# kemingy/rabitq

Measured on AMD Instinct MI355X. Metric: queries/sec at recall@10>=0.95, 100Mx128; HBM GB/s on popcount scan, higher is better.
Workload: dtype exact integer dot (fp6 MFMA, v_dot8_u32_u4) + f32

## Files before the change

### rabitq_amd/csrc/host_query.h

```cpp
#pragma once
struct QueryParams {
    uint32_t nq, len, probe, topk;
    bool heuristic;
    uint32_t cap, hcap;
    const float *thr_init = nullptr;
    bool seg_final = false;
    bool ext_lists = false;
    const rq_filter *filter = nullptr;
};

#define RQ_DEFAULT_CAP 4096u
#define RQ_MAX_CAP_HINT 32768u
#define RQ_MAX_NQ_PER_PASS 65536u
#define RQ_MAX_PROBE 16384u

static rq_status ws_prepare(const rq_index *idx, Workspace &ws, const QueryParams &qp) {
    const uint32_t nprobe = std::min(qp.probe, idx->k);
    const uint64_t nq = qp.nq, npairs = nq * nprobe;
    if (!ws.stream) HIPC(hipStreamCreateWithFlags(&ws.stream, hipStreamNonBlocking));
    if (!ws.h_totals) HIPC(hipHostMalloc((void **)&ws.h_totals, 16 * sizeof(unsigned long long)));
    RQC(ws.qpad.ensure(nq * idx->dim));
    RQC(ws.y.ensure(nq * idx->dim));
    if (!qp.ext_lists) RQC(ws.dist.ensure(nq * idx->k));
    RQC(ws.probe_dist.ensure(npairs));
// ... 21 lines not shown
    RQC(ws.heap_key.ensure(nq * qp.topk));
    RQC(ws.heap_id.ensure(nq * qp.topk));
    RQC(ws.precise.ensure(nq));
    RQC(ws.need.ensure(nq));
    RQC(ws.ovf.ensure(nq));
    RQC(ws.q_cap.ensure(nq));
    RQC(ws.q_base.ensure(nq));
    RQC(ws.nsurv.ensure(nq));
    RQC(ws.nshadow.ensure(nq));
    RQC(ws.recent.ensure(nq));
    RQC(ws.win_count.ensure(nq));
    RQC(ws.arr_len.ensure(nq));
    RQC(ws.row_map.ensure(nq));
    RQC(ws.big_list.ensure(nq + 3));
    if (qp.heuristic) RQC(ws.arr.ensure(nq * qp.hcap));
    return RQ_OK;
}

struct PassResult {
    uint64_t rough = 0, precise = 0, overflowed = 0, max_need = 0;
};

static rq_status finish_pass(const rq_index *idx, Workspace &ws, PassResult *res, rq_profile_t *prof_acc) {
    Prof &pf = ws.prof;
    const uint32_t nq = ws.pend_nq, dim = idx->dim;
    HIPC(hipStreamSynchronize(ws.stream));
    HIPC(hipGetLastError());
    res->rough = ws.h_totals[0];
    res->precise = ws.h_totals[1];
    res->overflowed = ws.h_totals[2];
    res->max_need = ws.h_totals[4];
    if (rq_large_batch(nq)) hints_of(idx, ws.pend_filter).big_dirs.store((uint32_t)ws.h_totals[7]);
    if (ws.pend_additive && ws.h_totals[8] >= 4096 && ws.h_totals[9] * 32 > ws.h_totals[8])
        const_cast<rq_index *>(idx)->additive_loose.store(1);
    if (prof_acc) prof_acc->matrix_subtile_steps += ws.h_totals[8], prof_acc->matrix_exact_steps += ws.h_totals[9];
    if (prof_acc) prof_acc->coarse_fallback_rows += (uint32_t)std::min<unsigned long long>(ws.h_totals[10], 0xFFFFFFFFull);
    if (pf.on && prof_acc) {
        float ms[PF_N] = {0};
        pf.collect(ms);
        prof_acc->ms_rotate += ms[PF_ROTATE], prof_acc->ms_coarse += ms[PF_COARSE];
        prof_acc->ms_select += ms[PF_SELECT], prof_acc->ms_prep += ms[PF_PREP], prof_acc->ms_group += ms[PF_GROUP];
        prof_acc->ms_scan += ms[PF_SCAN] + ms[PF_SCAN_MATRIX], prof_acc->ms_scan_matrix += ms[PF_SCAN_MATRIX];
        prof_acc->ms_rerank += ms[PF_RERANK], prof_acc->ms_sort += ms[PF_SORT];
        if (!ws.pend_matrix_ranges.empty()) {
            std::vector<unsigned long long> len(nq);
            HIPC(hipMemcpy(len.data(), ws.pend_filter ? ws.stream_len.p : ws.rough_cnt.p, (size_t)nq * 8, hipMemcpyDeviceToHost));
            for (const StreamRange &r : ws.pend_matrix_ranges)
                for (uint32_t b = 0; b < nq; ++b)
                    prof_acc->matrix_pairs += std::min<unsigned long long>(len[b], r.s_hi) - std::min<unsigned long long>(len[b], r.s_lo);
        }
        prof_acc->ms_replay += ms[PF_REPLAY], prof_acc->ms_total += ms[PF_TOTAL], prof_acc->ms_early += ms[PF_EARLY];
    }
    if (prof_acc) {
        const uint64_t slots = std::max<uint64_t>((uint64_t)nq * ws.pend_cap, ws.pend_seg_slots);
        prof_acc->survivor_workspace_bytes = std::max<uint64_t>(prof_acc->survivor_workspace_bytes,
            ws.pend_seg_slots ? (ws.surv.count + ws.runs.count + ws.runs_tmp.count + ws.arena_recs.count + ws.arena_runs.count) * 16ull
                              : slots * (ws.use_runs_tmp ? 48ull : 32ull));
        prof_acc->segmented_passes += ws.pend_seg_slots ? 1u : 0u;
        prof_acc->scan_candidates += res->rough;
        prof_acc->scan_bytes += res->rough * (uint64_t)(dim / 8 + 16);
        prof_acc->rerank_candidates += ws.h_totals[3];
        prof_acc->rerank_shadow_rejects += ws.h_totals[5];
        if (g_scan_dbg.load() & 256) {
            unsigned long long ht[12];
            HIPC(hipMemcpy(ht, ws.stat.p + 128, sizeof ht, hipMemcpyDeviceToHost));
            if (ht[3])
                fprintf(stderr, "[rabitq_hip] scan_mfma exact path (wave 0 of every block): %.0f cycles per block inside it (of which flushes %.0f), "
                        "%.1f flagged registers, %.1f with survivors and %.2f flushes per block\n", (double)ht[5] / ht[3], (double)ht[6] / ht[3],
                        (double)ht[9] / ht[3], (double)ht[7] / ht[3], (double)ht[8] / ht[3]);
            if (ht[3])
                fprintf(stderr, "[rabitq_hip] scan_mfma timing: %llu blocks, %.1f tiles/block; per block cycles: start-up %.0f, "
                        "tile-loop waits %.0f, tile bodies %.0f (per tile: wait %.0f, body %.0f)\n", ht[3], (double)ht[4] / ht[3],
                        (double)ht[0] / ht[3], (double)ht[1] / ht[3], (double)ht[2] / ht[3], (double)ht[1] / std::max(1ull, ht[4]),
                        (double)ht[2] / std::max(1ull, ht[4]));
        }
        if ((g_scan_dbg.load() & 4096) && nq <= RQ_SB_MAX_NQ) {
            unsigned long long hs[32];
            HIPC(hipMemcpy(hs, ws.stat.p, sizeof hs, hipMemcpyDeviceToHost));
            std::string line = "[rabitq_hip] sb_query_kernel phases (us since entry):";
            for (unsigned long long i = 1; i < std::min<unsigned long long>(hs[0], 30); ++i) line += " " + std::to_string((hs[1 + i] - hs[1]) / 100.0).substr(0, 6);
            fprintf(stderr, "%s\n", line.c_str());
        }
    }
    return RQ_OK;
}

static rq_status run_pass(const rq_index *idx, Workspace &ws, const float *d_q, const QueryParams &qp,
                          const uint32_t *d_row_map, float *d_out_dist, uint32_t *d_out_id, uint32_t *d_out_n,
                          PassResult *res, rq_profile_t *prof_acc, const uint32_t *ext_cluster = nullptr,
                          const float *ext_dist = nullptr, bool defer = false) {
    const uint32_t dim = idx->dim, k = idx->k, W = idx->W;
    const uint32_t nq = qp.nq, nprobe = std::min(qp.probe, k), topk = qp.topk;
    const uint32_t npairs = nq * nprobe;
    bool listed = false;
    uint32_t nlive = 0;
    const rq_filter *filt = qp.filter;
    ws.pend_filter = filt;
    const uint32_t min_len = filt ? 0u : idx->min_list_len;
    hipStream_t st = ws.stream;
    ws.pend_prefiltered = false;
    Prof &pf = ws.prof;
    pf.reset(g_profiling.load(), st);
    pf.begin(PF_TOTAL);
    size_t total_span = pf.spans.size() ? pf.spans.size() - 1 : 0;

    const int impl = g_scan_impl.load();
    struct Stage {
        uint32_t s_lo, s_hi;
    };
    auto build_stages = [&](uint64_t first_hi, uint64_t growth, uint64_t settle_cap) {
        std::vector<Stage> stages;
        const uint64_t total_max = std::min<uint64_t>((uint64_t)nprobe * idx->max_list_len, idx->n);
        uint64_t lo = 0, hi = first_hi;
        const uint64_t avg = std::max<uint64_t>(1, idx->n / std::max<uint32_t>(idx->nonempty_lists, 1));
        uint64_t settle = std::min(settle_cap, std::max<uint64_t>(avg, std::min<uint64_t>(idx->max_list_len, 16 * avg)));
        if (rq_large_batch(nq)) settle = std::max<uint64_t>(1, settle * (uint64_t)g_stage_settle_pct.load() / 100);
        while (lo < total_max) {
            const bool last = hi >= total_max || lo >= settle;
            stages.push_back({(uint32_t)lo, last ? 0xFFFFFFFFu : (uint32_t)hi});
            if (last) break;
            lo = hi;
            hi = std::min<uint64_t>(hi * growth, 0xFFFFFFF0ull);
            if (lo < 2 * avg && 2 * hi > 2 * avg) hi = 2 * avg;
            if (lo < settle && hi > settle) hi = settle;
        }
        return stages;
    };
    std::vector<Stage> stages;
    ReplayState rs;
    rs.thr = ws.thr.p, rs.heap_len = ws.heap_len.p, rs.heap_key = ws.heap_key.p, rs.heap_id = ws.heap_id.p;
    rs.precise = ws.precise.p, rs.need = ws.need.p, rs.nsurv = ws.nsurv.p, rs.nshadow = ws.nshadow.p, rs.recent_max = ws.recent.p, rs.win_count = ws.win_count.p;
    rs.arr_len = ws.arr_len.p, rs.arr = ws.arr.p, rs.hcap = qp.hcap;
    rs.ovf = ws.ovf.p;
    const QSeg useg{nullptr, nullptr, qp.cap};
    const float *qpad = d_q;
    const uint32_t *probe_cluster = ws.probe_cluster.p;
    const float *probe_dist = ws.probe_dist.p;
    const uint32_t *rerank_order = nullptr;
    const bool one_stage = qp.thr_init != nullptr && d_row_map == nullptr;
    auto stage_on_matrix = [&](const Stage &sg) {
        const uint64_t avg_len = std::max<uint64_t>(1, idx->n / std::max<uint32_t>(idx->nonempty_lists, 1));
        const uint64_t span = (uint64_t)std::min<uint64_t>(sg.s_hi, (uint64_t)nprobe * idx->max_list_len) - sg.s_lo;
        const uint64_t est_pairs = (uint64_t)nq * std::min<uint64_t>(nprobe, span / avg_len + 2);
        return scan_has_mfma(W) && impl != 1 &&
               (impl == 2 || (est_pairs >= 8ull * k && (sg.s_lo >= avg_len * (uint64_t)g_stage_settle_pct.load() / 100 || one_stage)));
    };

    const bool sb_w = W == 1 || W == 2 || W == 4 || W == 8 || W == 12 || W == 16;
    bool small = g_small_batch.load() == 0 && nq <= RQ_SB_MAX_NQ && !ext_cluster && !d_row_map && !qp.thr_init && !filt && sb_w &&
                 k <= RQ_SB_MAX_K && nprobe <= 64 && topk <= RQ_SB_MAX_TOPK && qp.cap <= 4 * RQ_DEFAULT_CAP;
    bool sb_results_done = false;
    bool sb_fused_finish = false;
    bool sb_filled = false;
    if (small) {
        const int gopt = g_stage_growth.load();
        stages = build_stages(16ull * std::max<uint32_t>(topk, 1), gopt >= 2 ? (uint64_t)gopt : 8, (uint64_t)std::max(1, g_sb_span.load()));
        if (stages.size() > RQ_SB_MAX_STAGES) small = false;
    }
    if (small) {
        const uint64_t total_max = std::min<uint64_t>((uint64_t)nprobe * idx->max_list_len, idx->n);
        SbArgs sa{};
        const bool whole = stages.empty() || (total_max - stages.back().s_lo) * (uint64_t)(dim / 8 + 16) <= (1ull << 20);
        sa.nstages = (uint32_t)(whole ? stages.size() : stages.size() - 1);
        for (uint32_t i = 0; i < sa.nstages; ++i) sa.s_lo[i] = stages[i].s_lo, sa.s_hi[i] = stages[i].s_hi;
        const Stage fin = whole ? Stage{0, 0} : stages.back();
        const uint64_t fin_pairs = (uint64_t)nq * nprobe;
        const bool fin_cluster_major = !whole && fin_pairs >= k / 2 && fin_pairs > 64;
        sa.finalize = whole ? 1u : 0u;
        sa.fill_final = !whole && !fin_cluster_major ? 1u : 0u;
        sa.final_lo = fin.s_lo;
        sa.codes = reinterpret_cast<const uint32_t *>(idx->codes.p), sa.factors = idx->factors.p, sa.centroids = idx->centroids.p;
        sa.offsets = idx->offsets.p, sa.map_ids = idx->map_ids.p, sa.base = idx->view();
        sa.dist = ws.dist.p, sa.y = ws.y.p, sa.qpad = ws.qpad.p, sa.probe_cluster = ws.probe_cluster.p, sa.probe_dist = ws.probe_dist.p;
        sa.qf6 = scan_has_mfma(W) && impl != 1 ? ws.qf6.p : nullptr;
        sa.scal = ws.scal.p, sa.qnib = ws.qnib.p, sa.rough_cnt = ws.rough_cnt.p, sa.surv_cnt = ws.surv_cnt.p, sa.totals = ws.totals.p;
        sa.rs = rs, sa.out_dist = d_out_dist, sa.out_id = d_out_id, sa.out_n = d_out_n, sa.recs = ws.recs.p, sa.fs = idx->fstats;
        sa.k = k, sa.dim = dim, sa.nprobe = nprobe, sa.topk = topk, sa.cap = qp.cap, sa.hcap = qp.hcap;
        sa.stamps = (g_scan_dbg.load() & 4096) ? ws.stat.p : nullptr;
        if (sa.stamps) HIPC(hipMemsetAsync(ws.stat.p, 0, 8, st));
        else HIPC(hipMemsetAsync(ws.stat.p, 0, 256 * sizeof(unsigned long long), st));
        pf.begin(PF_COARSE);
        sb_front_kernel<<<dim3(ceil_div(k, RQ_SB_LISTS), ceil_div(nq, RQ_SB_QT)), 256, (size_t)2 * RQ_SB_QT * dim * sizeof(float), st>>>(
            d_q, qp.len, idx->P.p, idx->centroids.p, ws.y.p, ws.qpad.p, ws.dist.p, k, dim, nq, ws.totals.p, ws.big_list.p + nq);
        pf.end();
        pf.begin(PF_EARLY);
        const size_t dyn = (size_t)RQ_SB_CAP * sizeof(SurvRec) + (size_t)dim * 4 + (size_t)topk * 16;
        const int mode = qp.heuristic ? 2 : (topk < 64 ? 1 : 0);
#define RQ_SBQ(WW)                                                                        \
    do {                                                                                  \
        if (mode == 2) sb_query_kernel<WW, 2><<<nq, 1024, dyn, st>>>(sa);                 \
        else if (mode == 1) sb_query_kernel<WW, 1><<<nq, 1024, dyn, st>>>(sa);            \
        else sb_query_kernel<WW, 0><<<nq, 1024, dyn, st>>>(sa);                           \
    } while (0)
        switch (W) {
            case 1: RQ_SBQ(1); break;
            case 2: RQ_SBQ(2); break;
            case 4: RQ_SBQ(4); break;
            case 8: RQ_SBQ(8); break;
            case 12: RQ_SBQ(12); break;
            default: RQ_SBQ(16); break;
        }
#undef RQ_SBQ
        pf.end();
        qpad = ws.qpad.p;
        sb_results_done = whole && !qp.heuristic;
        sb_fused_finish = !whole && !qp.heuristic;
        sb_filled = sa.fill_final != 0;
        stages.clear();
        if (!whole) stages.push_back(fin);
        if (prof_acc) prof_acc->small_batch_passes++;
    } else {
    pf.begin(PF_ROTATE);
    if (qp.len != dim) {
        pad_rows_kernel<<<ceil_div((uint64_t)nq * dim, 256), 256, 0, st>>>(d_q, ws.qpad.p, nq, qp.len, dim);
        qpad = ws.qpad.p;
    }
    launch_rotate(qpad, idx->P.p, ws.y.p, nq, dim, nq >= 32, st);
    pf.end();

    if (ext_cluster) {
        probe_cluster = ext_cluster;
        probe_dist = ext_dist;
    } else {
        if (coarse_prefilter_applies(idx, nq, nprobe)) {
            pf.begin(PF_COARSE);
            HIPC(hipMemsetAsync(ws.totals.p + 12, 0, 8, st));
            RQC(ws.coarse_redo.ensure(nq));
            RQC(ws.qf6.ensure((size_t)nq * dim / 2 + 16));
            launch_coarse_prefiltered(idx, ws.y.p, ws.dist.p, nq, nprobe, ws.probe_cluster.p, ws.probe_dist.p, nprobe, ws.totals.p + 12, ws.coarse_redo.p, st,
                                      reinterpret_cast<uint16_t *>(ws.qf6.p));
            ws.pend_prefiltered = true;
            pf.end();
        } else {
            pf.begin(PF_COARSE);
            launch_coarse(idx->cent_t.p, ws.y.p, ws.dist.p, k, dim, nq, k, st);
            pf.end();
            pf.begin(PF_SELECT);
            launch_select(ws.dist.p, k, nprobe, ws.probe_cluster.p, ws.probe_dist.p, 0, nprobe, nq, st);
            pf.end();
        }
    }

    if (one_stage) {
        stages.push_back({0u, 0xFFFFFFFFu});
    } else {
        const int gopt = g_stage_growth.load();
        const uint64_t growth = gopt >= 2 ? (uint64_t)gopt : (nq >= 32768 ? 8 : 16);
        stages = build_stages((uint64_t)std::max<uint32_t>(topk, 1) * (rq_large_batch(nq) ? growth : 1), growth, ~0ull);
    }
    pf.begin(PF_PREP);
    {
        uint32_t *qn = scan_is_fused(W) ? ws.qnib.p : nullptr;
        uint32_t *q6 = scan_has_mfma(W) && impl != 1 ? ws.qf6.p : nullptr;
        uint32_t qn_slots = nprobe;
        if (qn && q6 && !ext_cluster && min_len > 0) {
            uint32_t reach = 0;
            for (const Stage &sg : stages)
                if (!stage_on_matrix(sg))
                    reach = std::max<uint32_t>(reach, sg.s_hi == 0xFFFFFFFFu ? nprobe : (uint32_t)std::min<uint64_t>(nprobe, (uint64_t)(sg.s_hi - 1) / min_len + 1));
            qn_slots = reach;
        }
        listed = (filt || (idx->nonempty_lists * 2 < k && npairs >= 65536)) && g_pair_split.load() != 0 &&
                 (dim == 64 || dim == 128 || dim == 256 || dim == 512 || dim == 768 || dim == 1024);
        if (listed) {
            RQC(ws.live_list.ensure((size_t)npairs + 1));
            HIPC(hipMemsetAsync(ws.live_list.p + npairs, 0, 4, st));
            pair_split_kernel<<<ceil_div(npairs, 4096), 1024, 0, st>>>(filt ? filt->sub_off.p : idx->offsets.p, probe_cluster, probe_dist, npairs,
                                                                       nprobe, k, ws.scal.p, ws.live_list.p, ws.live_list.p + npairs);
            unsigned long long *h_live = ws.h_totals + 15;
            *h_live = 0;
            HIPC(hipMemcpyAsync(h_live, ws.live_list.p + npairs, 4, hipMemcpyDeviceToHost, st));
            HIPC(hipStreamSynchronize(st));
            nlive = (uint32_t)*h_live;
        }
#define RQ_PREP_SMALL(LP, R, PPB, PP)                                                                              \
    do {                                                                                                           \
        if (listed)                                                                                                \
            prep_small_listed_kernel<LP, R, PP><<<std::max(1u, ceil_div(nlive, (PPB) * (PP))), 256, 0, st>>>(ws.y.p, idx->centroids.p, idx->offsets.p, probe_cluster, \
                                                                    probe_dist, ws.live_list.p, nlive, nprobe, ws.scal.p, qn, q6, k); \
        else                                                                                                       \
            prep_small_kernel<LP, R, PP><<<ceil_div(npairs, (PPB) * (PP)), 256, 0, st>>>(ws.y.p, idx->centroids.p, idx->offsets.p, probe_cluster, \
                                                                    probe_dist, npairs, nprobe, ws.scal.p, qn, q6, k, idx->nonempty_lists * 2 < k ? 2u : 1u, qn_slots); \
    } while (0)
        if (dim == 128) RQ_PREP_SMALL(16, 2, 16, 2);
        else if (dim == 64) RQ_PREP_SMALL(16, 1, 16, 4);
        else if (dim == 256) RQ_PREP_SMALL(32, 2, 8, 2);
        else if (dim == 512) RQ_PREP_SMALL(32, 4, 8, 1);
        else if (dim == 768) RQ_PREP_SMALL(32, 6, 8, 1);
        else if (dim == 1024) RQ_PREP_SMALL(32, 8, 8, 1);
#undef RQ_PREP_SMALL
        else
            prep_kernel<<<ceil_div(npairs, 4), 256, 0, st>>>(ws.y.p, idx->centroids.p, idx->offsets.p, probe_cluster, probe_dist,
                                                             npairs, nprobe, dim, ws.scal.p,
                                                             scan_is_fused(W) ? nullptr : ws.planes.p,
                                                             qn, q6, nullptr, k, 1u);
    }
    if (filt) {
        RQC(ws.stream_len.ensure(nq));
        pair_prefix_filtered_kernel<<<ceil_div(nq, 4), 256, 0, st>>>(ws.scal.p, nq, nprobe, ws.rough_cnt.p, probe_cluster, filt->sub_off.p, k,
                                                                     ws.stream_len.p);
    } else
        pair_prefix_kernel<<<ceil_div(nq, 4), 256, 0, st>>>(ws.scal.p, nq, nprobe, ws.rough_cnt.p);
    if (rq_large_batch(nq)) {
        HIPC(hipMemsetAsync(ws.q_hist.p, 0, (size_t)(k + 2) * 4, st));
        order_count_kernel<<<ceil_div(nq, 256), 256, 0, st>>>(probe_cluster, nprobe, nq, k, ws.q_hist.p);
        group_scan_kernel<<<1, 1024, 0, st>>>(ws.q_hist.p, k + 1, ws.q_start.p, 0u, nullptr, 0u);
        order_scatter_kernel<<<ceil_div(nq, 256), 256, 0, st>>>(probe_cluster, nprobe, nq, k, ws.q_start.p, ws.q_hist.p,
                                                                ws.q_order.p);
        rerank_order = ws.q_order.p;
    }
    init_state_kernel<<<ceil_div(nq, 256), 256, 0, st>>>(rs, ws.surv_cnt.p, nq, qp.thr_init, d_row_map);
    HIPC(hipMemsetAsync(ws.totals.p, 0, 8 * sizeof(unsigned long long), st));
    HIPC(hipMemsetAsync(ws.big_list.p + nq, 0, 12, st));
    HIPC(hipMemsetAsync(ws.stat.p, 0, 256 * sizeof(unsigned long long), st));
    pf.end();

    }
    ws.pend_matrix_ranges.clear();
    ws.pend_seg_slots = 0;
    ws.pend_additive = false, ws.pend_matrix_stages = 0;
    const uint32_t big_hint = hints_of(idx, filt).big_dirs.load();
    const uint32_t mid_blocks = big_hint == 0 ? 64u : std::min(4096u, std::max(256u, big_hint / 4));
    const uint32_t tile = scan_tile(W);
    const uint64_t avg_len = std::max<uint64_t>(1, idx->n / std::max<uint32_t>(idx->nonempty_lists, 1));
    uint32_t stage_no = ~0u;
    for (const Stage &sg : stages) {
        ++stage_no;
        const uint64_t span = (uint64_t)std::min<uint64_t>(sg.s_hi, (uint64_t)nprobe * idx->max_list_len) - sg.s_lo;
        const uint64_t est_pairs = (uint64_t)nq * std::min<uint64_t>(nprobe, span / avg_len + 2);
        const bool use_mfma = stage_on_matrix(sg);
        const bool cluster_major = use_mfma || (est_pairs >= k / (small ? 2u : (uint32_t)g_cluster_major_div.load()) && est_pairs > 64);
        if (g_scan_dbg.load() & 16384)
            fprintf(stderr, "[rabitq_hip] stage %u: [%u, %u) span %llu est_pairs %llu %s\n", stage_no, sg.s_lo, sg.s_hi,
                    (unsigned long long)span, (unsigned long long)est_pairs, use_mfma ? "matrix cores" : (cluster_major ? "VALU, list-major" : "VALU, pair-major"));
        const bool fp6_records = use_mfma;
        const bool arena_stage = qp.seg_final && span > qp.cap && scan_is_fused(W) && rq_large_batch(nq);
        const int gate_opt = g_scan_gate.load();
        const bool additive = use_mfma && !arena_stage && !filt && scan_has_additive(W) && idx->list_uref.p != nullptr && gate_opt != 1 &&
                              (gate_opt == 2 || !idx->additive_loose.load());
        pf.begin(PF_GROUP);
        ScanArgs a{};
        ScanPtrs sp{};
        a.cluster_major = cluster_major ? 1u : 0u;
        uint32_t slot_hi = nprobe;
        if (cluster_major && min_len > 0 && !ext_cluster && sg.s_hi != 0xFFFFFFFFu)
            slot_hi = (uint32_t)std::min<uint64_t>(nprobe, (uint64_t)(sg.s_hi - 1) / min_len + 1);
        const uint32_t stage_pairs = nq * slot_hi;
        bool ranked = false;
        if (cluster_major) {
            HIPC(hipMemsetAsync(ws.grp_cnt.p, 0, (size_t)((k + 4) & ~3u) * 4, st));
            const int rank_opt = g_group_rank.load();
            ranked = k <= 32768 && (rank_opt == 2 || (rank_opt == 1 && stage_pairs >= 16 * RQ_RANK_ITEMS &&
                                                      stage_pairs / RQ_RANK_ITEMS >= k / 256));
            if (ranked) {
                const uint32_t nblk = ceil_div(stage_pairs, RQ_RANK_ITEMS);
                RQC(ws.pair_rank.ensure(stage_pairs));
                RQC(ws.rank_base.ensure((size_t)nblk * k));
                group_rank_kernel<<<nblk, 1024, (size_t)k * 4, st>>>(ws.scal.p, probe_cluster, stage_pairs, nprobe, slot_hi, sg.s_lo,
                                                                    sg.s_hi, k, ws.grp_cnt.p, ws.pair_rank.p, ws.rank_base.p);
            } else
                group_count_kernel<<<ceil_div(stage_pairs, 256), 256, 0, st>>>(ws.scal.p, probe_cluster, stage_pairs, nprobe,
                                                                               slot_hi, sg.s_lo, sg.s_hi, ws.grp_cnt.p);
            group_scan_kernel<<<1, 1024, 0, st>>>(ws.grp_cnt.p, k, ws.grp_start.p, (use_mfma ? 1u : 0u) | (ranked ? 2u : 0u) | (additive ? 4u : 0u), ws.recs.p, 12 * W);
            a.ngroups = k;
        } else {
            a.ngroups = npairs;
        }
        const uint32_t *operand = fp6_records ? ws.qf6.p
                                              : (scan_is_fused(W) ? ws.qnib.p : reinterpret_cast<const uint32_t *>(ws.planes.p));
        if (!(sb_filled && !cluster_major)) {
            const bool fill_listed = listed && ranked && cluster_major && slot_hi == nprobe;
            const uint32_t fill_items = fill_listed ? nlive : stage_pairs;
            const bool fill8 = !use_mfma || additive;
            if (fill_items) {
                if (fill8)
                    stage_fill_kernel<8><<<ceil_div(fill_items, 32), 256, 0, st>>>(ws.scal.p, probe_cluster, operand, ws.thr.p, fill_items,
                                                                    nprobe, slot_hi, fp6_records ? 12 * W : 8 * W, sg.s_lo, sg.s_hi,
                                                                    a.cluster_major, ws.grp_start.p, ws.grp_cnt.p, ws.recs.p,
                                                                    idx->fstats, use_mfma ? (additive ? 2u : 1u) : 0u, ranked ? ws.pair_rank.p : nullptr,
                                                                    ws.rank_base.p, k, idx->list_uref.p, fill_listed ? ws.live_list.p : nullptr);
                else
                    stage_fill_kernel<16><<<ceil_div(fill_items, 16), 256, 0, st>>>(ws.scal.p, probe_cluster, operand, ws.thr.p, fill_items,
                                                                    nprobe, slot_hi, fp6_records ? 12 * W : 8 * W, sg.s_lo, sg.s_hi,
                                                                    a.cluster_major, ws.grp_start.p, ws.grp_cnt.p, ws.recs.p,
                                                                    idx->fstats, use_mfma ? (additive ? 2u : 1u) : 0u, ranked ? ws.pair_rank.p : nullptr,
                                                                    ws.rank_base.p, k, idx->list_uref.p, fill_listed ? ws.live_list.p : nullptr);
            }
        }
        if (additive) {
            RQC(ws.grp_vref.ensure(2 * (size_t)k));
            group_vrange_kernel<<<k, 256, 0, st>>>(ws.recs.p, ws.grp_start.p, ws.grp_cnt.p, 12 * W, ws.grp_vref.p);
            ws.pend_additive = true;
        }
        pf.end();
        sp.codes = reinterpret_cast<const uint32_t *>(idx->codes.p);
        sp.factors = idx->factors.p;
        sp.grp_start = ws.grp_start.p;
        sp.grp_cnt = ws.grp_cnt.p;
        sp.offsets = idx->offsets.p;
        sp.recs = ws.recs.p;
        sp.surv = ws.surv.p;
        sp.runs = ws.runs.p;
        sp.surv_cnt = ws.surv_cnt.p;
        sp.stat = ws.stat.p;
        sp.list_uref = idx->list_uref.p, sp.grp_vref = ws.grp_vref.p;
        sp.arena = arena_stage, sp.filtered = filt != nullptr;
        a.x = filt ? filt->extra.p : nullptr;
        a.cap = qp.cap;
        a.dbg = (uint32_t)g_scan_dbg.load();
        const uint32_t stage_tile = use_mfma ? scan_mfma_tile(W, arena_stage, additive) : tile;
        a.tiles_per_group = ceil_div(std::min<uint64_t>(idx->max_list_len, sg.s_hi), stage_tile);
        sp.tile_table = nullptr;
        const uint64_t grid_blocks = (uint64_t)k * a.tiles_per_group, real_tiles = idx->n / stage_tile + k;
        const int tt_opt = g_scan_tile_table.load();
        if (cluster_major && scan_is_fused(W) && sg.s_hi >= idx->max_list_len &&
            (tt_opt == 2 || (tt_opt == 1 && grid_blocks > 4 * real_tiles))) {
            uint32_t count = 0;
            sp.tile_table = get_tile_table(idx, stage_tile, &count);
            if (sp.tile_table) a.use_table = 1u, a.ngroups = count, a.tiles_per_group = 1u;
        }
        uint32_t dense_cells = 0;
        if (rq_large_batch(nq) && !use_mfma && scan_is_fused(W) && g_dense_dir.load() && sg.s_hi != 0xFFFFFFFFu &&
            !(qp.seg_final && span > qp.cap)) {
            const uint64_t cells = (uint64_t)((sg.s_hi - 1) >> 6) - (sg.s_lo >> 6) + 2ull * slot_hi + 2;
            if (cells <= qp.cap) dense_cells = (uint32_t)cells;
        }
        a.dense_dir = dense_cells ? 1u : 0u;
        QSeg seg = useg;
        bool runs_in_tmp = false;
        if (arena_stage) {
            uint64_t want = std::max<uint64_t>(hints_of(idx, filt).arena.load(), (uint64_t)nq * qp.cap / 2);
            unsigned long long total_slots = 0;
            uint32_t arena_rsub = 0;
            bool arena_retried = false;
            ws.arena_failed = true;
#ifdef RQ_DEV_ABLATIONS
            if (g_seg_opt.load() == 3) {
                DevBuf<SurvRec> never;
                RQC(never.alloc(1ull << 46));
                return fail(RQ_ERR_OOM, "survivor arena: injected failure (developer hook survivor_segments = 3)");
            }
#endif
            for (int attempt = 0;; ++attempt) {
                want = std::min<uint64_t>(want, 0xFFFF0000ull);
                RQC(ws.arena_recs.ensure(want));
                RQC(ws.arena_runs.ensure(want));
                RQC(ws.arena_cur.ensure(RQ_ARENA_SHARDS + 4));
                RQC(ws.arena_fail.ensure(RQ_ARENA_SHARDS));
                HIPC(hipMemsetAsync(ws.arena_cur.p, 0, (RQ_ARENA_SHARDS + 4) * 8, st));
                HIPC(hipMemsetAsync(ws.arena_fail.p, 0xFF, RQ_ARENA_SHARDS * 4, st));
                ScanExtra hx{};
                RQC(ws.arena_places.ensure(want));
                hx.arena_places = ws.arena_places.p, hx.allow = filt ? filt->pos_bits.p : nullptr;
                hx.arena_recs = ws.arena_recs.p, hx.arena_runs = reinterpret_cast<uint4 *>(ws.arena_runs.p), hx.arena_cur = ws.arena_cur.p;
                hx.arena_fail = ws.arena_fail.p;
                {
                    const uint64_t have = std::min<uint64_t>(ws.arena_recs.count, ws.arena_runs.count);
                    hx.arena_sub = hx.arena_rsub = (uint32_t)(have * 7 / 8 / RQ_ARENA_SHARDS);
                    hx.arena_common = (uint32_t)std::min<uint64_t>(have - (uint64_t)hx.arena_sub * RQ_ARENA_SHARDS, 0xFFFFFF00ull);
                }
                arena_rsub = hx.arena_rsub;
                RQC(ws.scan_extra.ensure(1));
                HIPC(hipMemcpyAsync(ws.scan_extra.p, &hx, sizeof hx, hipMemcpyHostToDevice, st));
                a.x = ws.scan_extra.p;
                a.dense_dir = 0u;
                pf.begin(use_mfma ? PF_SCAN_MATRIX : PF_SCAN);
                if (use_mfma) launch_scan_mfma(sp, a, W, st, additive);
                else launch_scan(sp, a, W, st);
                pf.end();
                pf.begin(PF_GROUP);
                seg_exact_kernel<<<ceil_div(nq, 256), 256, 0, st>>>(ws.surv_cnt.p, nq, 64u, ws.q_cap.p);
                seg_scan_kernel<<<1, 1024, 0, st>>>(ws.q_cap.p, nq, ws.q_base.p, ws.arena_cur.p + RQ_ARENA_SHARDS + 1);
                unsigned long long tail[2] = {0, 0};
                HIPC(hipMemcpyAsync(tail, ws.arena_cur.p + RQ_ARENA_SHARDS, 16, hipMemcpyDeviceToHost, st));
                HIPC(hipStreamSynchronize(st));
                total_slots = tail[1];
                if (!(uint32_t)tail[0]) break;
                pf.end();
                if (attempt >= 6 || want >= 0xFFFF0000ull) return fail(RQ_ERR_OOM, "survivor arena kept overflowing");
                const uint64_t nblocks = a.use_table ? a.ngroups : (uint64_t)a.ngroups * a.tiles_per_group;
                HIPC(hipMemsetAsync(ws.surv_cnt.p, 0, (size_t)nq * sizeof(unsigned long long), st));
                want = std::max<uint64_t>(want * 2, 1u << 20);
                if (nblocks < RQ_ARENA_SHARDS) want = std::max<uint64_t>(want, 8 * total_slots + (1u << 16)), arena_retried = true;
                else want = std::max<uint64_t>(want, total_slots + total_slots / 4);
            }
            ws.arena_failed = false;
            {
                std::atomic<uint64_t> &arena_hint = hints_of(idx, filt).arena;
                uint64_t cur = arena_hint.load();
                const uint64_t learnt = std::max<uint64_t>(total_slots + total_slots * 3 / 5, arena_retried ? std::min<uint64_t>(want, 0xFFFF0000ull) : 0ull);
                while (cur < learnt && !arena_hint.compare_exchange_weak(cur, learnt)) {}
            }
            if (total_slots > ws.surv.count || total_slots > ws.runs.count || total_slots > ws.runs_tmp.count) {
                const uint64_t grow = total_slots + total_slots / 8;
                RQC(ws.surv.ensure(grow));
                RQC(ws.runs.ensure(grow));
                RQC(ws.runs_tmp.ensure(grow));
            }
            sp.surv = ws.surv.p, sp.runs = ws.runs.p;
            arena_scatter_kernel<<<dim3(RQ_ARENA_SHARDS + RQ_ARENA_COMMON_BLOCKS, 2), 256, 0, st>>>(ws.arena_recs.p, reinterpret_cast<const uint4 *>(ws.arena_runs.p), ws.arena_cur.p,
                                                                              ws.arena_fail.p, arena_rsub, ws.q_base.p, ws.arena_places.p, ws.surv.p, ws.runs_tmp.p);
            runs_in_tmp = true;
            pf.end();
            seg = QSeg{ws.q_base.p, ws.q_cap.p, qp.cap};
            ws.pend_seg_slots = std::max<uint64_t>(ws.pend_seg_slots, total_slots);
        }
        if (dense_cells) {
            pf.begin(PF_SORT);
            clear_dir_kernel<<<ceil_div((uint64_t)nq * dense_cells, 256), 256, 0, st>>>(ws.runs.p, nq, seg, dense_cells);
            pf.end();
        }
        if (!arena_stage) {
            pf.begin(use_mfma ? PF_SCAN_MATRIX : PF_SCAN);
            if (use_mfma) launch_scan_mfma(sp, a, W, st, additive);
            else launch_scan(sp, a, W, st);
            pf.end();
        }
        if (use_mfma) ws.pend_matrix_stages++;
        if (prof_acc && additive) prof_acc->matrix_additive_launches++;
        if (prof_acc) prof_acc->scan_launches++;
        if (prof_acc && use_mfma) {
            prof_acc->matrix_launches++;
            ws.pend_matrix_ranges.push_back({sg.s_lo, sg.s_hi});
        }
        if (!rq_large_batch(nq) && qp.cap <= 4 * RQ_DEFAULT_CAP) {
            pf.begin(PF_RERANK);
            const uint32_t fin_threads = nq <= 16 ? 1024u : 256u;
            const uint32_t presorted = qp.cap > RQ_DEFAULT_CAP && nprobe <= 1024 ? 1u : 0u;
            if (presorted) {
                sort_runs_kernel<<<nq, 64, 0, st>>>(ws.runs.p, ws.surv_cnt.p, seg, ws.big_list.p, ws.big_list.p + nq, RQ_SORT_LDS_RECS, nullptr);
                sort_runs_mid_kernel<<<std::min(nq, 256u), 256, RQ_SORT_MID_LDS_WORDS * 8, st>>>(ws.runs.p, ws.use_runs_tmp ? ws.runs_tmp.p : nullptr, ws.surv_cnt.p,
                                                                                              seg, ws.big_list.p, ws.big_list.p + nq, nprobe, 0u,
                                                                                              RQ_SORT_MID_LDS_WORDS);
            }
            if (sb_fused_finish) {
                uint32_t flags = presorted;
                if (nq <= 32) {
                    accurate_kernel<<<dim3(std::max(1u, std::min(16u, 256u / nq)), nq), 256, (size_t)dim * sizeof(float), st>>>(
                        ws.surv.p, ws.surv_cnt.p, seg, idx->view(), qpad, dim, nullptr, probe_cluster, nprobe);
                    flags |= 2u;
                }
                const uint32_t presorted = flags;
                if (topk < 64)
                    sb_finish_kernel<true><<<nq, fin_threads, (size_t)dim * sizeof(float) + (2 * RQ_SBF_RUNS + RQ_SBF_RECS) * 16, st>>>(
                        ws.surv.p, ws.runs.p, ws.surv_cnt.p, seg, idx->view(), qpad, dim, topk, rs, probe_cluster, nprobe, presorted,
                        idx->map_ids.p, d_out_dist, d_out_id, d_out_n, ws.rough_cnt.p, ws.totals.p);
                else
                    sb_finish_kernel<false><<<nq, fin_threads, (size_t)dim * sizeof(float) + (2 * RQ_SBF_RUNS + RQ_SBF_RECS) * 16, st>>>(
                        ws.surv.p, ws.runs.p, ws.surv_cnt.p, seg, idx->view(), qpad, dim, topk, rs, probe_cluster, nprobe, presorted,
                        idx->map_ids.p, d_out_dist, d_out_id, d_out_n, ws.rough_cnt.p, ws.totals.p);
                sb_results_done = true;
            } else if (qp.heuristic)
                stage_finish_kernel<true><<<nq, fin_threads, (size_t)dim * sizeof(float), st>>>(ws.surv.p, ws.runs.p, ws.surv_cnt.p, seg, idx->view(),
// ... 462 lines not shown
```

### rabitq_amd/csrc/host_state.h

```cpp
#pragma once
static thread_local std::string g_err;
static rq_status fail(rq_status s, const std::string &msg) {
    g_err = msg;
    return s;
}
#define HIPC(expr)                                                                                   \
    do {                                                                                             \
        hipError_t _e = (expr);                                                                      \
        if (_e != hipSuccess)                                                                        \
            return fail(_e == hipErrorOutOfMemory ? RQ_ERR_OOM : RQ_ERR_HIP,                         \
                        std::string(#expr) + ": " + hipGetErrorString(_e));                          \
    } while (0)
#define RQC(expr)                        \
    do {                                 \
        rq_status _s = (expr);           \
        if (_s != RQ_OK) return _s;      \
    } while (0)

static rq_status ensure_device() {
    int count = 0;
    hipError_t e = hipGetDeviceCount(&count);
    if (e != hipSuccess || count == 0)
        return fail(RQ_ERR_NO_DEVICE, "no HIP device visible (librabitq_hip has no CPU fallback)");
    return RQ_OK;
}

template <typename T>
struct DevBuf {
    T *p = nullptr;
    size_t count = 0;
    DevBuf() = default;
    DevBuf(const DevBuf &) = delete;
    DevBuf &operator=(const DevBuf &) = delete;
    ~DevBuf() { release(); }
    void release() {
        if (p) (void)hipFree(p);
        p = nullptr;
        count = 0;
    }
    rq_status alloc(size_t n) {
        release();
        count = n;
        if (n == 0) n = 1;
        hipError_t e = hipMalloc((void **)&p, n * sizeof(T));
        if (e != hipSuccess) {
            p = nullptr;
            count = 0;
            return fail(RQ_ERR_OOM, "hipMalloc of " + std::to_string(n * sizeof(T)) + " bytes failed: " +
                                        hipGetErrorString(e));
        }
        return RQ_OK;
    }
    rq_status ensure(size_t n) { return n <= count && p ? RQ_OK : alloc(n); }
};

template <typename T>
static rq_status copy_out_sized(T *out, T full) {
    const uint32_t sz = out->struct_size;
    if (sz < 8) return fail(RQ_ERR_INVALID, "struct_size is not set (set it to sizeof(the struct) before the call)");
    const uint32_t w = std::min<uint32_t>(sz, (uint32_t)sizeof(T));
    full.struct_size = w;
    memcpy(out, &full, w);
    return RQ_OK;
}
static inline uint32_t ceil_div(uint64_t a, uint64_t b) { return (uint32_t)((a + b - 1) / b); }
template <int W, int NT>
static size_t assign_lds_bytes() { return 2 * (32 * (64 * W * 2 + 16) + 128); }
static inline uint32_t pow2_ceil(uint32_t v) {
    uint32_t p = 1;
    while (p < v) p <<= 1;
    return p;
}

static std::atomic<uint64_t> g_rough{0}, g_precise{0}, g_query{0}, g_miss{0};

enum { PF_ROTATE = 0, PF_COARSE, PF_SELECT, PF_PREP, PF_GROUP, PF_SCAN, PF_SCAN_MATRIX, PF_RERANK, PF_SORT, PF_REPLAY, PF_EARLY, PF_TOTAL, PF_N };
static std::atomic<int> g_profiling{0};
static thread_local rq_profile_t g_profile;

struct Prof {
    bool on = false;
    bool light = false;
    hipStream_t stream = nullptr;
    struct Span {
        hipEvent_t a, b;
        int cat;
    };
    std::vector<Span> spans;
    std::vector<hipEvent_t> pool;
    size_t used = 0;
    bool open = false;
    hipEvent_t last_b = nullptr;
    bool failed = false;
    hipEvent_t get() {
        if (used == pool.size()) {
            hipEvent_t e = nullptr;
            if (hipEventCreate(&e) != hipSuccess || !e) {
                failed = true;
                on = false;
                return nullptr;
            }
            pool.push_back(e);
        }
        return pool[used++];
    }
    void begin(int cat) {
        open = on && !(light && cat != PF_SCAN && cat != PF_SCAN_MATRIX && cat != PF_TOTAL);
        if (!open) {
            last_b = nullptr;
            return;
        }
        Span s{last_b, get(), cat};
        if (s.b && !s.a) {
            s.a = get();
            if (s.a) (void)hipEventRecord(s.a, stream);
        }
        last_b = nullptr;
        if (!s.a || !s.b) {
            open = false;
            spans.clear();
            return;
        }
        spans.push_back(s);
    }
    void end() {
        if (!open) return;
        (void)hipEventRecord(spans.back().b, stream);
        last_b = spans.back().b;
        open = false;
    }
    void reset(int level, hipStream_t st) {
        on = level != 0;
        light = level == 2;
        stream = st;
        spans.clear();
        used = 0;
        open = false;
        last_b = nullptr;
        failed = false;
    }
    void collect(float *ms ) {
        if (failed) return;
        for (auto &s : spans) {
            float t = 0;
            (void)hipEventElapsedTime(&t, s.a, s.b);
            ms[s.cat] += t;
        }
    }
    ~Prof() {
        for (auto e : pool) (void)hipEventDestroy(e);
    }
};

struct StreamRange {
    uint32_t s_lo, s_hi;
};
struct Workspace {
    hipStream_t stream = nullptr;
    bool busy = false;
    size_t pend_total_span = 0;
    uint64_t pend_seg_slots = 0;
    uint32_t pend_cap = 0;
    uint32_t pend_nq = 0;
    std::vector<StreamRange> pend_matrix_ranges;
    DevBuf<float> qpad, y, dist, probe_dist, thr, recent;
    DevBuf<float> retry_q, retry_pd, retry_pc;
    DevBuf<uint32_t> retry_rows;
    DevBuf<uint32_t> q_hist, q_start, q_order;
    DevBuf<uint32_t> live_list;
    DevBuf<uint32_t> coarse_redo;
    DevBuf<uint32_t> pair_rank, rank_base;
    DevBuf<uint32_t> probe_cluster, recs, grp_cnt, grp_start, heap_len, heap_id, precise, need,
        nsurv, nshadow, win_count, arr_len, row_map, big_list;
    DevBuf<int32_t> heap_key;
    DevBuf<PairScalars> scal;
    DevBuf<uint64_t> planes;
    DevBuf<uint32_t> qnib;
    DevBuf<uint32_t> qf6;
    DevBuf<unsigned long long> rough_cnt, totals, surv_cnt, stat;
    DevBuf<unsigned long long> stream_len;
    const struct rq_filter *pend_filter = nullptr;
    DevBuf<float4> grp_vref;
    bool pend_additive = false;
    uint32_t pend_matrix_stages = 0;
    bool pend_prefiltered = false;
    DevBuf<SurvRec> surv, arr;
    DevBuf<RunRec> runs, runs_tmp;
    bool use_runs_tmp = false;
    bool arena_failed = false;
    DevBuf<float> sh_dist;
    DevBuf<uint32_t> sh_id, sh_n;
    DevBuf<unsigned long long> sh_packed, sh_gathered, sh_merged;
    DevBuf<uint32_t> ovf, q_cap;
    DevBuf<unsigned long long> q_base;
    DevBuf<SurvRec> arena_recs;
    DevBuf<RunRec> arena_runs;
    DevBuf<uint2> arena_places;
    DevBuf<unsigned long long> arena_cur;
    DevBuf<unsigned int> arena_fail;
    DevBuf<ScanExtra> scan_extra;
    DevBuf<uint32_t> sh_flag;
    DevBuf<uint32_t> sh_pc, sh_id_b, sh_n_b;
    DevBuf<float> sh_pd, sh_thr, sh_dist_b;
    unsigned long long *h_totals = nullptr;
    Prof prof;
    ~Workspace() {
        if (h_totals) (void)hipHostFree(h_totals);
        if (stream) (void)hipStreamDestroy(stream);
    }
};

struct rq_index {
    uint32_t dim = 0, k = 0, W = 0, max_list_len = 0;
    uint32_t min_list_len = 0;
    uint64_t n = 0;
    uint64_t n_dev = 0;
    float *base_host = nullptr;
    float *base_host_dev = nullptr;
    DevBuf<ListTier> list_tier;
    std::vector<ListTier> h_list_tier;
    bool split_rows = false;
    BaseView view() const { return BaseView{base.p, base_host_dev, list_tier.p, k, split_rows ? 1u : 0u}; }
    ~rq_index() {
        if (base_host) (void)hipHostFree(base_host);
    }
    DevBuf<float> base, P, centroids, cent_t;
    DevBuf<_Float16> base_h;
    DevBuf<uint8_t> base_q8;
    DevBuf<float4> list_q8;
    DevBuf<uint32_t> offsets, map_ids;
    DevBuf<uint64_t> codes;
    DevBuf<float4> factors;
    DevBuf<float4> list_uref;
    DevBuf<uint16_t> cent_bf;
    DevBuf<float> cent_sqnorm;
    float cent_norm_max = INFINITY;
    uint32_t nonempty_lists = 0;
    std::atomic<int> additive_loose{0};
    std::mutex ws_mu;
    std::vector<std::unique_ptr<Workspace>> ws_pool;
    FactorStats fstats{0, 0, 0, 0};
    std::atomic<uint32_t> cap_hint{0};
    std::atomic<uint64_t> arena_hint{0};
    std::atomic<uint32_t> big_dirs_hint{0};
    uint64_t pass_budget = 24ull << 30;
    std::vector<uint32_t> h_offsets;
    std::mutex tt_mu;
    std::map<uint32_t, std::unique_ptr<DevBuf<uint4>>> tile_tables;
    DevBuf<uint32_t> row_key;
    bool row_key_valid = false;
    bool row_order_ok = true;
    bool is_shard = false;
    uint64_t generation = 0;
    std::atomic<int> open_tickets{0};
};

struct rq_filter {
    const rq_index *idx = nullptr;
    uint64_t generation = 0;
    DevBuf<uint32_t> pos_bits;
    DevBuf<uint32_t> sub_off;
    DevBuf<ScanExtra> extra;
    uint64_t rows = 0;
    std::atomic<uint32_t> cap_hint{0};
    std::atomic<uint64_t> arena_hint{0};
    std::atomic<uint32_t> big_dirs_hint{0};
};
struct PassHints {
    std::atomic<uint32_t> &cap;
    std::atomic<uint64_t> &arena;
    std::atomic<uint32_t> &big_dirs;
};
static PassHints hints_of(const rq_index *idx, const rq_filter *f) {
    if (f) {
        rq_filter *m = const_cast<rq_filter *>(f);
        return PassHints{m->cap_hint, m->arena_hint, m->big_dirs_hint};
    }
    rq_index *m = const_cast<rq_index *>(idx);
    return PassHints{m->cap_hint, m->arena_hint, m->big_dirs_hint};
}

__global__ void fill_f32_kernel(float *p, float v, uint64_t n) {
    uint64_t i = (uint64_t)blockIdx.x * blockDim.x + threadIdx.x;
    if (i < n) p[i] = v;
}
__global__ void gather_rows_kernel(const float *__restrict__ in, const uint32_t *__restrict__ rows,
                                   uint32_t nrows, uint32_t len, float *__restrict__ out) {
    uint64_t i = (uint64_t)blockIdx.x * blockDim.x + threadIdx.x;
    if (i >= (uint64_t)nrows * len) return;
    uint32_t r = (uint32_t)(i / len), c = (uint32_t)(i - (uint64_t)r * len);
    out[i] = in[(uint64_t)rows[r] * len + c];
}

__global__ __launch_bounds__(256) void shard_gather_kernel(const uint32_t *__restrict__ new_off, const uint32_t *__restrict__ old_off,
                                                           uint32_t k, uint64_t n_local, uint32_t dim,
                                                           const BaseView base_in, const uint64_t *__restrict__ codes_in,
                                                           const float4 *__restrict__ factors_in, const uint32_t *__restrict__ ids_in,
                                                           const BaseView base_out, uint64_t *__restrict__ codes_out,
                                                           float4 *__restrict__ factors_out, uint32_t *__restrict__ ids_out) {
    const uint32_t lane = threadIdx.x & 63, W = dim >> 6;
    for (uint64_t p = (uint64_t)blockIdx.x * 4 + (threadIdx.x >> 6); p < n_local; p += (uint64_t)gridDim.x * 4) {
        uint32_t lo = 0, hi = k;
        while (hi - lo > 1) {
            const uint32_t mid = lo + ((hi - lo) >> 1);
            if (new_off[mid] <= p) lo = mid;
            else hi = mid;
        }
        const uint64_t src = (uint64_t)old_off[lo] + (p - new_off[lo]);
        const RowRef srow = base_in.row(src, dim), drow = base_out.row(p, dim);
        for (uint32_t e = lane; e < dim; e += 64) rq_row_put(drow, dim, e, rq_row_get(srow, dim, e));
        for (uint32_t w = lane; w < W; w += 64) codes_out[p * W + w] = codes_in[src * W + w];
        if (lane == 0) {
            factors_out[p] = factors_in[src];
            ids_out[p] = ids_in[src];
        }
    }
}
__global__ void pack_topk_keys_kernel(const float *__restrict__ dist, const uint32_t *__restrict__ id, const uint32_t *__restrict__ cnt,
                                      uint32_t nq, uint32_t topk, uint32_t id_offset, unsigned long long *__restrict__ keys) {
    const uint64_t i = (uint64_t)blockIdx.x * blockDim.x + threadIdx.x;
    if (i >= (uint64_t)nq * topk) return;
    const uint32_t b = (uint32_t)(i / topk), e = (uint32_t)(i - (uint64_t)b * topk);
    keys[i] = e < cnt[b] ? (((unsigned long long)ord32_biased(dist[i]) << 32) | (uint32_t)(id[i] + id_offset)) : ~0ull;
}
// ... 57 lines not shown
                                                                                                    kstride);
}

static std::atomic<int> g_pair_split{1};
static std::atomic<int> g_coarse_tiled_from{4096};
static bool coarse_prefilter_has(uint32_t W) { return W == 1 || W == 2 || W == 3 || W == 4 || W == 6 || W == 8 || W == 12; }
static bool coarse_prefilter_applies(const rq_index *idx, uint32_t nq, uint32_t nprobe) {
    const int impl = g_coarse_impl.load();
    return (impl == 3 || impl == 4 || (impl == 0 && nq >= 2048)) && coarse_prefilter_has(idx->W) && std::isfinite(idx->cent_norm_max) &&
           idx->cent_bf.p != nullptr && nprobe <= 64 && nq >= 8 && idx->k >= 64 && nprobe >= 1 && idx->k <= 65536;
}
static void launch_coarse_prefiltered(const rq_index *idx, const float *y, float *dist, uint32_t nq, uint32_t nprobe, uint32_t *out_cluster,
                                      float *out_dist, uint32_t out_stride, unsigned long long *fallback_rows, uint32_t *redo, hipStream_t st,
                                      uint16_t *y_bf) {
    const uint32_t k = idx->k, dim = idx->dim;
    if (idx->W > 8) to_bf16_kernel<<<ceil_div((uint64_t)nq * dim / 8, 256), 256, 0, st>>>(y, (uint64_t)nq * dim, y_bf);
#define RQ_CAP(WW, NT)                                                                                                      \
    coarse_approx_kernel<WW, NT><<<ceil_div(nq, 128 * NT), 256, assign_lds_bytes<WW, NT>(), st>>>(y, idx->cent_bf.p, idx->cent_sqnorm.p, nq, \
                                                                                                  k, dist, y_bf)
    switch (idx->W) {
        case 1: RQ_CAP(1, 2); break;
        case 2: RQ_CAP(2, 2); break;
        case 3: RQ_CAP(3, 1); break;
        case 4: RQ_CAP(4, 1); break;
        case 6: RQ_CAP(6, 1); break;
        case 8: RQ_CAP(8, 1); break;
        default: RQ_CAP(12, 1); break;
    }
#undef RQ_CAP
    const dim3 g(ceil_div(nq, 4)), b(256);
    const uint32_t ntile = ceil_div(k, 32u);
    const int impl = g_coarse_impl.load();
    const bool tiled = redo != nullptr && ntile >= nprobe &&
                       (k > 8192 || impl == 4 || (impl != 3 && k >= (uint32_t)g_coarse_tiled_from.load() && idx->W <= 8));
    if (tiled) {
#define RQ_TILED(TPL)                                                                                                             \
    select_refine_tiled_kernel<TPL><<<g, b, 4 * 64 * (TPL) * 4, st>>>(dist, y, idx->centroids.p, idx->cent_norm_max, k, dim, nprobe, out_cluster, \
                                                                    out_dist, out_stride, nq, redo, fallback_rows)
        if (ntile <= 128) RQ_TILED(2);
        else if (ntile <= 256) RQ_TILED(4);
        else if (ntile <= 512) RQ_TILED(8);
        else if (ntile <= 1024) RQ_TILED(16);
        else RQ_TILED(32);
#undef RQ_TILED
        select_probe_kernel<<<nq, 256, (size_t)nprobe * 8, st>>>(dist, k, nprobe, out_cluster, out_dist, 0u, out_stride, redo);
    } else if (k <= 1024)
        select_refine_wave_kernel<16><<<g, b, 0, st>>>(dist, y, idx->centroids.p, idx->cent_norm_max, k, dim, nprobe, out_cluster, out_dist, out_stride, nq, fallback_rows);
    else if (k <= 4096)
        select_refine_wave_kernel<64><<<g, b, 0, st>>>(dist, y, idx->centroids.p, idx->cent_norm_max, k, dim, nprobe, out_cluster, out_dist, out_stride, nq, fallback_rows);
    else
        select_refine_wave_kernel<128><<<g, b, 0, st>>>(dist, y, idx->centroids.p, idx->cent_norm_max, k, dim, nprobe, out_cluster, out_dist, out_stride, nq, fallback_rows);
}

#define RQ_MAX_BLOCKS_256 ((1u << 23) - 1)

static void launch_rotate(const float *x, const float *P, float *out, uint64_t n, uint32_t dim, bool mfma,
                          hipStream_t st) {
    const uint64_t rows_per_launch = mfma ? (1ull << 40) : (uint64_t)RQ_MAX_BLOCKS_256 * 4;
    for (uint64_t r0 = 0; r0 < n; r0 += rows_per_launch) {
        const uint64_t m = std::min(rows_per_launch, n - r0);
        const float *xs = x + r0 * dim;
        float *os = out + r0 * dim;
        if (mfma) {
            const uint32_t ncol = dim / ROT_BN;
            const uint64_t nrow_tiles = ceil_div(m, ROT_BM);
            const uint32_t groups = (uint32_t)std::min<uint64_t>(nrow_tiles, std::max<uint32_t>(1, 512 / ncol));
            rotate_mfma_kernel<<<dim3(groups * ncol), dim3(256), 0, st>>>(xs, P, os, m, dim, groups);
        } else {
            rotate_valu_kernel<<<dim3(ceil_div(m, 4), dim / 64), dim3(64, 4), 0, st>>>(xs, P, os, m, dim);
        }
    }
}

static const uint4 *get_tile_table(const rq_index *cidx, uint32_t tile, uint32_t *count) {
    rq_index *idx = const_cast<rq_index *>(cidx);
    std::lock_guard<std::mutex> lk(idx->tt_mu);
    auto it = idx->tile_tables.find(tile);
    if (it == idx->tile_tables.end()) {
        std::vector<uint4> h;
        h.reserve(idx->n / tile + idx->k + 1);
        for (uint32_t c = 0; c < idx->k; ++c) {
            const uint32_t b = idx->h_offsets[c], len = idx->h_offsets[c + 1] - b;
            for (uint32_t f = 0; f < len; f += tile) h.push_back(make_uint4(c, f, b, len));
        }
        std::unique_ptr<DevBuf<uint4>> buf(new DevBuf<uint4>());
        if (buf->alloc(h.size()) != RQ_OK) return nullptr;
        if (!h.empty() && hipMemcpy(buf->p, h.data(), h.size() * sizeof(uint4), hipMemcpyHostToDevice) != hipSuccess) return nullptr;
        buf->count = h.size();
        it = idx->tile_tables.emplace(tile, std::move(buf)).first;
    }
    *count = (uint32_t)it->second->count;
    return it->second->p;
}

static std::atomic<uint32_t> g_max_scan_blocks{RQ_MAX_BLOCKS_256};
template <typename F>
static void launch_scan_chunks(const ScanArgs &a, F &&launch) {
    if (a.ngroups == 0 || a.tiles_per_group == 0) return;
    const uint32_t maxb = std::max(1u, g_max_scan_blocks.load());
    const uint32_t tchunk = std::min(a.tiles_per_group, maxb);
    const uint32_t gchunk = std::max(1u, maxb / tchunk);
    for (uint32_t t0 = 0; t0 < a.tiles_per_group; t0 += tchunk)
        for (uint32_t g0 = 0; g0 < a.ngroups; g0 += gchunk) {
            ScanArgs c = a;
            c.tile_base = t0, c.group_base = g0;
            c.tiles_per_group = std::min(tchunk, a.tiles_per_group - t0);
            c.ngroups = std::min(gchunk, a.ngroups - g0);
            launch(c, dim3(c.ngroups * c.tiles_per_group));
        }
}

#define SCAN_ARGS p.codes, p.factors, p.offsets, p.grp_start, p.recs, p.surv, p.runs, p.surv_cnt, p.tile_table, a
template <bool ARENA, bool FILT>
static void launch_scan_t(const ScanPtrs &p, const ScanArgs &args, uint32_t W, hipStream_t st) {
    launch_scan_chunks(args, [&](const ScanArgs &a, dim3 g) {
        const dim3 b(256);
#define RQ_SCAN_K(WW, CPL)                                                                        \
    do {                                                                                          \
        if constexpr (FILT) scan_kernel<WW, CPL, ARENA, true><<<g, b, 0, st>>>(SCAN_ARGS);         \
        else scan_kernel<WW, CPL, ARENA><<<g, b, 0, st>>>(SCAN_ARGS);                             \
    } while (0)
        switch (W) {
            case 1: RQ_SCAN_K(1, 2); break;
            case 2: RQ_SCAN_K(2, 2); break;
            case 3: RQ_SCAN_K(3, 2); break;
            case 4: RQ_SCAN_K(4, 2); break;
            case 6: RQ_SCAN_K(6, 2); break;
            case 8: RQ_SCAN_K(8, 2); break;
            case 12: RQ_SCAN_K(12, 1); break;
            case 16: RQ_SCAN_K(16, 1); break;
            default:
                if constexpr (!ARENA && FILT) scan_generic_filtered_kernel<<<g, b, 0, st>>>(SCAN_ARGS, W);
                else if constexpr (!ARENA) scan_generic_kernel<<<g, b, 0, st>>>(SCAN_ARGS, W);
                break;
        }
#undef RQ_SCAN_K
    });
}
static void launch_scan(const ScanPtrs &p, const ScanArgs &args, uint32_t W, hipStream_t st) {
    if (p.filtered) {
        if (p.arena) launch_scan_t<true, true>(p, args, W, st);
        else launch_scan_t<false, true>(p, args, W, st);
    } else if (p.arena) launch_scan_t<true, false>(p, args, W, st);
    else launch_scan_t<false, false>(p, args, W, st);
}
static std::atomic<int> g_scan_impl{0};
static std::atomic<int> g_scan_gate{0};
static std::atomic<int> g_stage_growth{0};
static std::atomic<int> g_large_from{256};
static bool rq_large_batch(uint32_t nq) { return nq >= (uint32_t)g_large_from.load(); }
static std::atomic<int> g_cluster_major_div{32};
static std::atomic<int> g_stage_settle_pct{100};
static std::atomic<int> g_scan_tile_table{1};
static std::atomic<int> g_group_rank{1};
static std::atomic<int> g_shared_thr{1};
static std::atomic<int> g_sb_span{2560};
static std::atomic<int> g_seg_opt{1};
static std::atomic<int> g_pass_overlap{1};
static std::atomic<int> g_small_batch{0};
static std::atomic<int> g_dense_dir{1};

static bool scan_has_mfma(uint32_t W) {
    switch (W) {
        case 1: case 2: case 3: case 4: case 6: case 8: case 12: case 16: return true;
        default: return false;
    }
}
static uint32_t scan_mfma_nt(uint32_t W, bool additive = false) { return W == 2 ? (additive ? RQ_ADD_NT2 : RQ_NT_W2) : (W == 12 ? RQ_NT_W12 : (W >= 4 ? 2 : 4)); }
static uint32_t scan_mfma_nw(uint32_t W, bool arena) { return W == 2 && !arena ? 8u : 4u; }
static uint32_t scan_mfma_tile(uint32_t W, bool arena, bool additive = false) { return 32 * scan_mfma_nw(W, arena) * scan_mfma_nt(W, additive && !arena); }
static size_t scan_mfma_ring_bytes(uint32_t W, bool arena = false) {
    (void)arena;
    const uint64_t slots = W <= 2 ? 4ull : (W >= 16 ? 5ull : 3ull);
    return slots * (32 * (12 * W + 2) + RQ_REC_TAIL * 32) * 4;
}
template <int W, int NT, bool ARENA, bool ADD = false, bool FILT = false>
static void launch_scan_mfma_t(const ScanPtrs &p, const ScanArgs &a, dim3 g, hipStream_t st) {
    scan_mfma_kernel<W, NT, ARENA, ADD, FILT><<<g, dim3(64 * scan_mfma_waves<W, ARENA>()), scan_mfma_ring_bytes(W, ARENA), st>>>(p.codes, p.factors, p.offsets, p.grp_start, p.grp_cnt,
                                                                                    p.recs, p.surv, p.runs, p.surv_cnt, p.stat, p.tile_table, p.list_uref, p.grp_vref, a);
}
static bool scan_has_additive(uint32_t W) { return W == 1 || W == 2; }
static void launch_scan_mfma_add(const ScanPtrs &p, const ScanArgs &args, uint32_t W, hipStream_t st) {
    launch_scan_chunks(args, [&](const ScanArgs &a, dim3 g) {
        switch (W) {
            case 1: launch_scan_mfma_t<1, 4, false, true>(p, a, g, st); break;
            case 2: launch_scan_mfma_t<2, RQ_ADD_NT2, false, true>(p, a, g, st); break;
            default: break;
        }
    });
}
template <bool ARENA, bool FILT = false>
static void launch_scan_mfma_a(const ScanPtrs &p, const ScanArgs &args, uint32_t W, hipStream_t st) {
    launch_scan_chunks(args, [&](const ScanArgs &a, dim3 g) {
        switch (W) {
            case 1: launch_scan_mfma_t<1, 4, ARENA, false, FILT>(p, a, g, st); break;
            case 2: launch_scan_mfma_t<2, RQ_NT_W2, ARENA, false, FILT>(p, a, g, st); break;
            case 3: launch_scan_mfma_t<3, 4, ARENA, false, FILT>(p, a, g, st); break;
            case 4: launch_scan_mfma_t<4, 2, ARENA, false, FILT>(p, a, g, st); break;
            case 6: launch_scan_mfma_t<6, 2, ARENA, false, FILT>(p, a, g, st); break;
            case 8: launch_scan_mfma_t<8, 2, ARENA, false, FILT>(p, a, g, st); break;
            case 12: launch_scan_mfma_t<12, RQ_NT_W12, ARENA, false, FILT>(p, a, g, st); break;
            case 16: launch_scan_mfma_t<16, 2, ARENA, false, FILT>(p, a, g, st); break;
            default: break;
        }
    });
}
static void launch_scan_mfma(const ScanPtrs &p, const ScanArgs &args, uint32_t W, hipStream_t st, bool additive = false) {
    if (p.filtered) {
        if (p.arena) launch_scan_mfma_a<true, true>(p, args, W, st);
        else launch_scan_mfma_a<false, true>(p, args, W, st);
    } else if (p.arena) launch_scan_mfma_a<true>(p, args, W, st);
    else if (additive) launch_scan_mfma_add(p, args, W, st);
    else launch_scan_mfma_a<false>(p, args, W, st);
}

static bool scan_is_fused(uint32_t W) {
    switch (W) {
        case 1: case 2: case 3: case 4: case 6: case 8: case 12: case 16: return true;
        default: return false;
    }
}
static uint32_t scan_tile(uint32_t W) {
    switch (W) {
        case 1: case 2: case 3: case 4: case 6: case 8: return 512;
        default: return 256;
    }
}

static void launch_select(const float *dist, uint32_t k, uint32_t nprobe, uint32_t *out_cluster, float *out_dist,
                          uint32_t id_offset, uint32_t out_stride, uint32_t nq, hipStream_t st) {
    if (select_is_wave(k, nprobe, nq)) {
        const dim3 g(ceil_div(nq, 4)), b(256);
        if (k <= 1024) select_probe_wave_kernel<16><<<g, b, 0, st>>>(dist, k, nprobe, out_cluster, out_dist, id_offset, out_stride, nq);
        else if (k <= 4096) select_probe_wave_kernel<64><<<g, b, 0, st>>>(dist, k, nprobe, out_cluster, out_dist, id_offset, out_stride, nq);
        else select_probe_wave_kernel<128><<<g, b, 0, st>>>(dist, k, nprobe, out_cluster, out_dist, id_offset, out_stride, nq);
        return;
    }
    select_probe_kernel<<<nq, 256, (size_t)nprobe * 8, st>>>(dist, k, nprobe, out_cluster, out_dist, id_offset, out_stride);
}

template <int W, int NT>
static hipError_t set_scan_mfma_attr() {
    hipError_t e = hipFuncSetAttribute(reinterpret_cast<const void *>(scan_mfma_kernel<W, NT, false>),
                                       hipFuncAttributeMaxDynamicSharedMemorySize, (int)scan_mfma_ring_bytes(W));
    if (e != hipSuccess) return e;
    if constexpr (W <= 2) {
        e = hipFuncSetAttribute(reinterpret_cast<const void *>(scan_mfma_kernel<W, (W == 2 ? RQ_ADD_NT2 : NT), false, true>),
                                hipFuncAttributeMaxDynamicSharedMemorySize, (int)scan_mfma_ring_bytes(W));
        if (e != hipSuccess) return e;
    }
    e = hipFuncSetAttribute(reinterpret_cast<const void *>(scan_mfma_kernel<W, NT, true>),
                            hipFuncAttributeMaxDynamicSharedMemorySize, (int)scan_mfma_ring_bytes(W));
    if (e != hipSuccess) return e;
    e = hipFuncSetAttribute(reinterpret_cast<const void *>(scan_mfma_kernel<W, NT, false, false, true>),
                            hipFuncAttributeMaxDynamicSharedMemorySize, (int)scan_mfma_ring_bytes(W));
    if (e != hipSuccess) return e;
    return hipFuncSetAttribute(reinterpret_cast<const void *>(scan_mfma_kernel<W, NT, true, false, true>),
                               hipFuncAttributeMaxDynamicSharedMemorySize, (int)scan_mfma_ring_bytes(W));
}
static rq_status ensure_kernel_attributes() {
    static std::once_flag once;
    static hipError_t err = hipSuccess;
    static const char *what = "";
    std::call_once(once, [] {
        auto set = [&](const void *fn, int bytes, const char *name) {
            if (err != hipSuccess) return;
            err = hipFuncSetAttribute(fn, hipFuncAttributeMaxDynamicSharedMemorySize, bytes);
            if (err != hipSuccess) what = name;
        };
        set(reinterpret_cast<const void *>(select_probe_kernel), 140 * 1024, "select_probe_kernel");
        set(reinterpret_cast<const void *>(coarse_dist_kernel<4>), 140 * 1024, "coarse_dist_kernel<4>");
        set(reinterpret_cast<const void *>(coarse_dist_kernel<8>), 140 * 1024, "coarse_dist_kernel<8>");
        set(reinterpret_cast<const void *>(assign_generic_kernel<8>), 140 * 1024, "assign_generic_kernel<8>");
        set(reinterpret_cast<const void *>(merge_smallest_u64_kernel), 16384 * 8, "merge_smallest_u64_kernel");
        set(reinterpret_cast<const void *>(group_rank_kernel), 32768 * 4, "group_rank_kernel");
        set(reinterpret_cast<const void *>(sb_front_kernel), 140 * 1024, "sb_front_kernel");
        set(reinterpret_cast<const void *>(sort_runs_mid_kernel), RQ_SORT_MID_LDS_WORDS * 8, "sort_runs_mid_kernel");
        set(reinterpret_cast<const void *>(assign_approx_kernel<6, 1>), (int)assign_lds_bytes<6, 1>(), "assign_approx_kernel<6,1>");
        set(reinterpret_cast<const void *>(assign_approx_kernel<8, 1>), (int)assign_lds_bytes<8, 1>(), "assign_approx_kernel<8,1>");
        set(reinterpret_cast<const void *>(assign_approx_kernel<12, 1>), (int)assign_lds_bytes<12, 1>(), "assign_approx_kernel<12,1>");
        set(reinterpret_cast<const void *>(coarse_approx_kernel<6, 1>), (int)assign_lds_bytes<6, 1>(), "coarse_approx_kernel<6,1>");
        set(reinterpret_cast<const void *>(coarse_approx_kernel<8, 1>), (int)assign_lds_bytes<8, 1>(), "coarse_approx_kernel<8,1>");
        set(reinterpret_cast<const void *>(coarse_approx_kernel<12, 1>), (int)assign_lds_bytes<12, 1>(), "coarse_approx_kernel<12,1>");
        set(reinterpret_cast<const void *>(sb_finish_kernel<true>), 104 * 1024, "sb_finish_kernel");
        set(reinterpret_cast<const void *>(sb_finish_kernel<false>), 104 * 1024, "sb_finish_kernel");
#define RQ_SBQ_ATTR(WW)                                                                                  \
    set(reinterpret_cast<const void *>(sb_query_kernel<WW, 0>), 120 * 1024, "sb_query_kernel");          \
    set(reinterpret_cast<const void *>(sb_query_kernel<WW, 1>), 120 * 1024, "sb_query_kernel");          \
    set(reinterpret_cast<const void *>(sb_query_kernel<WW, 2>), 120 * 1024, "sb_query_kernel")
        RQ_SBQ_ATTR(1);
        RQ_SBQ_ATTR(2);
        RQ_SBQ_ATTR(4);
        RQ_SBQ_ATTR(8);
        RQ_SBQ_ATTR(12);
        RQ_SBQ_ATTR(16);
#undef RQ_SBQ_ATTR
        auto chk = [&](hipError_t e, const char *name) {
            if (err == hipSuccess && e != hipSuccess) err = e, what = name;
        };
        chk(set_scan_mfma_attr<1, 4>(), "scan_mfma_kernel<1,4>");
        chk(set_scan_mfma_attr<2, RQ_NT_W2>(), "scan_mfma_kernel<2,NT>");
        chk(set_scan_mfma_attr<3, 4>(), "scan_mfma_kernel<3,4>");
        chk(set_scan_mfma_attr<4, 2>(), "scan_mfma_kernel<4,2>");
        chk(set_scan_mfma_attr<6, 2>(), "scan_mfma_kernel<6,2>");
        chk(set_scan_mfma_attr<8, 2>(), "scan_mfma_kernel<8,2>");
        chk(set_scan_mfma_attr<12, RQ_NT_W12>(), "scan_mfma_kernel<12,NT>");
// ... 8 lines not shown
```

### rabitq_amd/csrc/kernels_query.h

```cpp
#pragma once
#ifndef RQ_COLLECT_UNROLL
#define RQ_COLLECT_UNROLL 8
#endif
#include "common.h"
#include "kernels_scan_common.h"

#pragma clang fp contract(off)

__global__ void pad_rows_kernel(const float *__restrict__ in, float *__restrict__ out, uint64_t n,
                                uint32_t len, uint32_t dim) {
    uint64_t i = (uint64_t)blockIdx.x * blockDim.x + threadIdx.x;
    if (i >= n * dim) return;
    uint64_t r = i / dim;
    uint32_t c = (uint32_t)(i - r * dim);
    out[i] = c < len ? in[r * len + c] : 0.0f;
}

__global__ __launch_bounds__(256) void rotate_valu_kernel(const float *__restrict__ x,
                                                          const float *__restrict__ P,
                                                          float *__restrict__ out, uint64_t n,
                                                          uint32_t dim) {
    uint64_t r = (uint64_t)blockIdx.x * 4 + threadIdx.y;
    uint32_t j = blockIdx.y * 64 + threadIdx.x;
    if (r >= n) return;
// ... 694 lines not shown
                for (int i = 0; i < (int)(RQ_COARSE_CAND / 64); ++i) c += (uint32_t)__popcll(__ballot(kk[i] <= mid));
                if (c >= nprobe) {
                    h2 = mid;
                    if (c <= nprobe + 12) break;
                } else {
                    l2 = mid + 1;
                }
            }
            T2 = coarse_margin_key(yr, dim, cmax, ord32_unbias(h2));
            ok = T2 != 0xFFFFFFFFu && collect(T2);
        }
    }
    if (!ok || base < nprobe) {
        for (uint32_t j0 = 0; j0 < k; j0 += 32) {
            uint32_t jj[4];
            float ee[4];
#pragma unroll
            for (int q = 0; q < 4; ++q) jj[q] = j0 + 8 * q + grp < k ? j0 + 8 * q + grp : 0u;
            coarse_exact_dist4(centroids, yr, dim, al, jj, ee);
#pragma unroll
            for (int q = 0; q < 4; ++q)
                if (j0 + 8 * q + grp < k && al == 0) d[j0 + 8 * q + grp] = ee[q];
        }
        if (lane == 0) {
            redo_flag[b] = 1u;
            if (fallback_rows) atomicAdd(fallback_rows, 1ull);
        }
        return;
    }
    if (lane == 0) redo_flag[b] = 0u;
    __builtin_amdgcn_fence(__ATOMIC_SEQ_CST, "wavefront");
    coarse_refine_tail(wn, base, centroids, yr, dim, nprobe, b, out_cluster, out_dist, out_stride);
}

__global__ __launch_bounds__(256) void merge_smallest_u64_kernel(const unsigned long long *__restrict__ in, uint32_t world,
                                                                 uint32_t nq, uint32_t width, uint32_t m_out,
                                                                 unsigned long long *__restrict__ out, uint64_t rank_stride) {
    extern __shared__ __attribute__((aligned(16))) unsigned char merge_smem[];
    unsigned long long *keys = reinterpret_cast<unsigned long long *>(merge_smem);
    const uint32_t b = blockIdx.x, m = world * width;
    for (uint32_t i = threadIdx.x; i < m; i += blockDim.x) {
        const uint32_t w = i / width, e = i - w * width;
        keys[i] = in[(uint64_t)w * rank_stride + (uint64_t)b * width + e];
    }
    __syncthreads();
    bitonic_sort_block(keys, m, [](unsigned long long v) { return v; });
    for (uint32_t i = threadIdx.x; i < m_out; i += blockDim.x) out[(uint64_t)b * m_out + i] = i < m ? keys[i] : ~0ull;
}

__global__ __launch_bounds__(256) void prep_kernel(const float *__restrict__ y,
                                                   const float *__restrict__ centroids,
                                                   const uint32_t *__restrict__ offsets,
                                                   const uint32_t *__restrict__ pair_cluster,
                                                   const float *__restrict__ pair_ycd, uint32_t npairs,
                                                   uint32_t pairs_per_row, uint32_t dim,
                                                   PairScalars *__restrict__ scal,
                                                   uint64_t *__restrict__ planes,
                                                   uint32_t *__restrict__ qnib,
                                                   uint32_t *__restrict__ qf6,
                                                   uint32_t *__restrict__ out_sum_u32, uint32_t nlists,
                                                   uint32_t skip_empty) {
    const uint32_t lane = threadIdx.x & 63;
    const uint32_t p = blockIdx.x * 4 + (threadIdx.x >> 6);
    if (p >= npairs) return;
    const uint32_t row = p / pairs_per_row;
    const uint32_t c = pair_cluster[p];
    const uint32_t len_c = c < nlists ? offsets[c + 1] - offsets[c] : 0u;
    if (len_c == 0 && skip_empty) {
        if (lane == 0) {
            PairScalars s;
            s.lower = 0.0f, s.delta = 0.0f, s.sumq = 0.0f, s.ycd = pair_ycd[p], s.ycd_sqrt = 0.0f;
            s.row = row, s.list_begin = 0, s.list_len = 0, s.stream_begin = 0, s.pad = 0;
            scal[p] = s;
            if (out_sum_u32) out_sum_u32[p] = 0;
        }
        return;
    }
    const float *yr = y + (uint64_t)row * dim;
    const float *cr = centroids + (uint64_t)c * dim;
    const uint32_t W = dim >> 6;
    float mn = 3.402823466e+38f, mx = -3.402823466e+38f;
    for (uint32_t w = 0; w < W; ++w) {
        float r = yr[64 * w + lane] - cr[64 * w + lane];
        mn = r < mn ? r : mn;
        mx = r > mx ? r : mx;
    }
    for (int o = 32; o >= 1; o >>= 1) {
        float a = __shfl_xor(mn, o, 64), bb = __shfl_xor(mx, o, 64);
        mn = a < mn ? a : mn;
        mx = bb > mx ? bb : mx;
    }
    const float scalar = 1.0f / 15.0f;
    const float delta = (mx - mn) * scalar;
    const float one_over_delta = 1.0f / delta;
    uint32_t sum = 0;
    uint64_t *pl = planes + (uint64_t)p * 4 * W;
    for (uint32_t w = 0; w < W; ++w) {
        float r = yr[64 * w + lane] - cr[64 * w + lane];
        int32_t q = cvtps_epi32((r - mn) * one_over_delta);
        sum += (uint32_t)q;
        if (planes) {
#pragma unroll
            for (int bit = 0; bit < 4; ++bit) {
                uint64_t word = __ballot((q >> bit) & 1);
                if (lane == 0) pl[bit * W + w] = word;
            }
        }
        if (qf6) {
            const uint32_t v = (uint32_t)q & 15u;
            const uint32_t c6 = v < 4 ? 4 * v : (v < 8 ? 8 + 2 * v : 16 + v);
            const uint32_t i16 = lane & 15, bitpos = 6 * i16, d0 = bitpos >> 5, off = bitpos & 31;
            const uint64_t wide = (uint64_t)c6 << off;
            const uint32_t lo32 = (uint32_t)wide, hi32 = (uint32_t)(wide >> 32);
            uint32_t w0 = d0 == 0 ? lo32 : 0u;
            uint32_t w1 = d0 == 0 ? hi32 : (d0 == 1 ? lo32 : 0u);
            uint32_t w2 = d0 == 1 ? hi32 : (d0 == 2 ? lo32 : 0u);
#pragma unroll
            for (int o = 1; o < 16; o <<= 1) {
                w0 |= __shfl_xor(w0, o, 16);
                w1 |= __shfl_xor(w1, o, 16);
                w2 |= __shfl_xor(w2, o, 16);
            }
            if (i16 < 3)
                qf6[(uint64_t)p * 12 * W + (lane >> 5) * 6 * W + 6 * w + 3 * ((lane >> 4) & 1) + i16] =
                    i16 == 0 ? w0 : (i16 == 1 ? w1 : w2);
        }
        if (qnib) {
            uint32_t nib = ((uint32_t)q & 15u) << (4 * (lane & 7));
            nib |= __shfl_xor(nib, 1, 8);
            nib |= __shfl_xor(nib, 2, 8);
            nib |= __shfl_xor(nib, 4, 8);
            if ((lane & 7) == 0) qnib[(uint64_t)p * 8 * W + 8 * w + (lane >> 3)] = nib;
        }
    }
    for (int o = 32; o >= 1; o >>= 1) sum += __shfl_xor(sum, o, 64);
    if (lane == 0) {
        PairScalars s;
        float ycd = pair_ycd[p];
        s.lower = mn;
        s.delta = delta;
        s.sumq = (float)sum;
        s.ycd = ycd;
        s.ycd_sqrt = sqrtf(ycd);
        s.row = row;
        s.list_begin = offsets[c];
        s.list_len = offsets[c + 1] - offsets[c];
        s.stream_begin = 0;
        s.pad = 0;
        scal[p] = s;
        if (out_sum_u32) out_sum_u32[p] = sum;
    }
}

template <int LP, int R, int PP>
__device__ __forceinline__ void prep_small_pairs(const float *__restrict__ y, const float *__restrict__ centroids,
                                                 const uint32_t *__restrict__ offsets,
                                                 const uint32_t *__restrict__ pair_cluster,
                                                 const float *__restrict__ pair_ycd, uint32_t npairs,
                                                 uint32_t pairs_per_row, PairScalars *__restrict__ scal,
                                                 uint32_t *__restrict__ qnib, uint32_t *__restrict__ qf6,
                                                 uint32_t nlists, uint32_t skip_empty, uint32_t p0,
                                                 const uint32_t *__restrict__ live_list = nullptr ,
                                                 uint32_t qn_slots = 0xFFFFFFFFu ) {
    static_assert(R >= 1 && (LP == 16 || LP == 32 || LP == 64), "lane groups of 16 / 32 / 64; a round = 4 LP dimensions (the packing's neighbour exchanges stay inside a round)");
    constexpr uint32_t DIM = 4 * LP * R, W = DIM / 64, PPW = 64 / LP;
    const uint32_t lane = threadIdx.x & 63, sub = lane % LP;
    uint32_t cl[PP], lb[PP], ll[PP];
    float ycd_in[PP];
    bool live[PP];
    uint32_t pid[PP];
#pragma unroll
    for (int pp = 0; pp < PP; ++pp) {
        const uint32_t pi = p0 + pp * PPW;
        live[pp] = pi < npairs;
        pid[pp] = live_list ? (live[pp] ? live_list[pi] : 0u) : pi;
        const uint32_t p = pid[pp];
        cl[pp] = live[pp] ? pair_cluster[p] : 0xFFFFFFFFu;
        ycd_in[pp] = live[pp] ? pair_ycd[p] : 0.0f;
    }
    float4 cv[PP][R], yv[PP][R];
#pragma unroll
    for (int pp = 0; pp < PP; ++pp) {
        const uint32_t p = pid[pp], c = cl[pp];
        const bool in = live[pp] && c < nlists;
        lb[pp] = in ? offsets[c] : 0u;
        ll[pp] = in ? offsets[c + 1] - lb[pp] : 0u;
        const uint32_t row = live[pp] ? p / pairs_per_row : 0u;
        const bool fetch = skip_empty == 2 ? ll[pp] != 0 : true;
#pragma unroll
        for (int rd = 0; rd < R; ++rd) {
            if (fetch) {
                yv[pp][rd] = *reinterpret_cast<const float4 *>(y + (uint64_t)row * DIM + 4 * LP * rd + 4 * sub);
                cv[pp][rd] = *reinterpret_cast<const float4 *>(centroids + (uint64_t)(in ? c : 0u) * DIM + 4 * LP * rd + 4 * sub);
            } else {
                yv[pp][rd] = make_float4(0.0f, 0.0f, 0.0f, 0.0f), cv[pp][rd] = make_float4(0.0f, 0.0f, 0.0f, 0.0f);
            }
        }
    }
#pragma unroll
    for (int pp = 0; pp < PP; ++pp) {
        const uint32_t p = pid[pp];
        if (!live[pp]) continue;
        const uint32_t row = p / pairs_per_row;
        if (ll[pp] == 0 && skip_empty) {
            if (sub == 0) {
                PairScalars s;
                s.lower = 0.0f, s.delta = 0.0f, s.sumq = 0.0f, s.ycd = ycd_in[pp], s.ycd_sqrt = 0.0f;
                s.row = row, s.list_begin = 0, s.list_len = 0, s.stream_begin = 0, s.pad = 0;
                scal[p] = s;
            }
            continue;
        }
        float r[R][4];
        float mn = 3.402823466e+38f, mx = -3.402823466e+38f;
#pragma unroll
        for (int rd = 0; rd < R; ++rd) {
            r[rd][0] = yv[pp][rd].x - cv[pp][rd].x, r[rd][1] = yv[pp][rd].y - cv[pp][rd].y;
            r[rd][2] = yv[pp][rd].z - cv[pp][rd].z, r[rd][3] = yv[pp][rd].w - cv[pp][rd].w;
#pragma unroll
            for (int e = 0; e < 4; ++e) {
                mn = r[rd][e] < mn ? r[rd][e] : mn;
                mx = r[rd][e] > mx ? r[rd][e] : mx;
            }
        }
#pragma unroll
        for (int o = LP / 2; o >= 1; o >>= 1) {
            const float a = __shfl_xor(mn, o, LP), bb = __shfl_xor(mx, o, LP);
            mn = a < mn ? a : mn;
            mx = bb > mx ? bb : mx;
        }
        const float scalar = 1.0f / 15.0f;
        const float delta = (mx - mn) * scalar;
        const float one_over_delta = 1.0f / delta;
        uint32_t sum = 0;
#pragma unroll
        for (int rd = 0; rd < R; ++rd) {
            uint32_t nib16 = 0, f24 = 0;
#pragma unroll
            for (int e = 0; e < 4; ++e) {
                const int32_t q = cvtps_epi32((r[rd][e] - mn) * one_over_delta);
                sum += (uint32_t)q;
                const uint32_t v = (uint32_t)q & 15u;
                nib16 |= v << (4 * e);
                f24 |= (v < 4 ? 4 * v : (v < 8 ? 8 + 2 * v : 16 + v)) << (6 * e);
            }
            const uint32_t dsub = LP * rd + sub;
            {
                const uint32_t other = __shfl_xor(nib16, 1, LP);
                if (qnib && (sub & 1) == 0 && p - row * pairs_per_row < qn_slots) qnib[(uint64_t)p * 8 * W + (dsub >> 1)] = nib16 | (other << 16);
            }
            {
                const uint32_t nxt = __shfl_down(f24, 1, LP);
                const uint32_t t = dsub & 7, sh = 8 * (t & 3);
                if (qf6 && (t & 3) != 3) {
                    const uint32_t w = dsub >> 4, h = (dsub >> 3) & 1;
                    qf6[(uint64_t)p * 12 * W + h * 6 * W + 6 * w + 3 * (t >> 2) + (t & 3)] = (f24 >> sh) | (nxt << (24 - sh));
                }
            }
        }
#pragma unroll
        for (int o = LP / 2; o >= 1; o >>= 1) sum += __shfl_xor(sum, o, LP);
        if (sub == 0) {
            PairScalars s;
            s.lower = mn;
            s.delta = delta;
            s.sumq = (float)sum;
            s.ycd = ycd_in[pp];
            s.ycd_sqrt = sqrtf(ycd_in[pp]);
            s.row = row;
            s.list_begin = lb[pp];
            s.list_len = ll[pp];
            s.stream_begin = 0;
            s.pad = 0;
            scal[p] = s;
        }
    }
}

template <int LP, int R, int PP>
__global__ __launch_bounds__(256) void prep_small_kernel(const float *__restrict__ y,
                                                         const float *__restrict__ centroids,
                                                         const uint32_t *__restrict__ offsets,
                                                         const uint32_t *__restrict__ pair_cluster,
                                                         const float *__restrict__ pair_ycd, uint32_t npairs,
                                                         uint32_t pairs_per_row, PairScalars *__restrict__ scal,
                                                         uint32_t *__restrict__ qnib, uint32_t *__restrict__ qf6,
                                                         uint32_t nlists, uint32_t skip_empty, uint32_t qn_slots) {
    constexpr uint32_t PPW = 64 / LP;
    const uint32_t p0 = (blockIdx.x * 4 + (threadIdx.x >> 6)) * (PPW * PP) + (threadIdx.x & 63) / LP;
    prep_small_pairs<LP, R, PP>(y, centroids, offsets, pair_cluster, pair_ycd, npairs, pairs_per_row, scal, qnib, qf6, nlists,
                                skip_empty, p0, nullptr, qn_slots);
}

__global__ __launch_bounds__(1024) void pair_split_kernel(const uint32_t *__restrict__ offsets, const uint32_t *__restrict__ pair_cluster,
                                                          const float *__restrict__ pair_ycd, uint32_t npairs, uint32_t pairs_per_row,
                                                          uint32_t nlists, PairScalars *__restrict__ scal,
                                                          uint32_t *__restrict__ live_list, uint32_t *__restrict__ live_count) {
    __shared__ uint32_t wcnt[4][16], s_base;
    const uint32_t lane = threadIdx.x & 63, wave = threadIdx.x >> 6;
    bool keep[4];
    uint32_t rank[4];
#pragma unroll
    for (int u = 0; u < 4; ++u) {
        const uint32_t p = blockIdx.x * 4096 + u * 1024 + threadIdx.x;
        keep[u] = false;
        if (p < npairs) {
            const uint32_t c = pair_cluster[p];
            const uint32_t len = c < nlists ? offsets[c + 1] - offsets[c] : 0u;
            keep[u] = len != 0;
            if (!keep[u]) {
                PairScalars s;
                s.lower = 0.0f, s.delta = 0.0f, s.sumq = 0.0f, s.ycd = pair_ycd[p], s.ycd_sqrt = 0.0f;
                s.row = p / pairs_per_row, s.list_begin = 0, s.list_len = 0, s.stream_begin = 0, s.pad = 0;
                scal[p] = s;
            }
        }
        const uint64_t m = __ballot(keep[u]);
        rank[u] = (uint32_t)__popcll(m & ((1ull << lane) - 1ull));
        if (lane == 0) wcnt[u][wave] = (uint32_t)__popcll(m);
    }
    __syncthreads();
    if (threadIdx.x == 0) {
        uint32_t tot = 0;
        for (int u = 0; u < 4; ++u)
            for (int w = 0; w < 16; ++w) {
                const uint32_t c = wcnt[u][w];
                wcnt[u][w] = tot;
                tot += c;
            }
        s_base = tot ? atomicAdd(live_count, tot) : 0u;
    }
    __syncthreads();
#pragma unroll
    for (int u = 0; u < 4; ++u)
        if (keep[u]) live_list[s_base + wcnt[u][wave] + rank[u]] = blockIdx.x * 4096 + u * 1024 + threadIdx.x;
}
template <int LP, int R, int PP>
__global__ __launch_bounds__(256) void prep_small_listed_kernel(const float *__restrict__ y,
                                                                const float *__restrict__ centroids,
                                                                const uint32_t *__restrict__ offsets,
                                                                const uint32_t *__restrict__ pair_cluster,
                                                                const float *__restrict__ pair_ycd, const uint32_t *__restrict__ live_list,
                                                                uint32_t nlive,
                                                                uint32_t pairs_per_row, PairScalars *__restrict__ scal,
                                                                uint32_t *__restrict__ qnib, uint32_t *__restrict__ qf6,
                                                                uint32_t nlists) {
    constexpr uint32_t PPW = 64 / LP;
    const uint32_t p0 = (blockIdx.x * 4 + (threadIdx.x >> 6)) * (PPW * PP) + (threadIdx.x & 63) / LP;
    prep_small_pairs<LP, R, PP>(y, centroids, offsets, pair_cluster, pair_ycd, nlive, pairs_per_row, scal, qnib, qf6, nlists, 1u, p0, live_list);
}

__device__ __forceinline__ void pair_prefix_row(PairScalars *__restrict__ scal, uint32_t b, uint32_t nprobe,
                                                unsigned long long *__restrict__ rough_count,
                                                const uint32_t *__restrict__ pair_cluster = nullptr,
                                                const uint32_t *__restrict__ sub_off = nullptr, uint32_t nlists = 0,
                                                unsigned long long *__restrict__ stream_len = nullptr) {
    const uint32_t lane = threadIdx.x & 63;
    unsigned long long carry = 0, admitted = 0;
    for (uint32_t s0 = 0; s0 < nprobe; s0 += 64) {
        const uint32_t s = s0 + lane;
        PairScalars *ps = scal + (uint64_t)b * nprobe + s;
        const unsigned long long len = s < nprobe ? ps->list_len : 0;
        unsigned long long incl = len;
#pragma unroll
        for (int o = 1; o < 64; o <<= 1) {
            const unsigned long long up = __shfl_up(incl, o, 64);
            if ((int)lane >= o) incl += up;
        }
        const unsigned long long begin = carry + incl - len;
        if (s < nprobe) ps->stream_begin = begin > 0xFFFFFFFFull ? 0xFFFFFFFFu : (uint32_t)begin;
        carry += __shfl(incl, 63, 64);
        if (sub_off) {
            const uint32_t c = s < nprobe && len ? pair_cluster[(uint64_t)b * nprobe + s] : 0xFFFFFFFFu;
            unsigned long long ad = c < nlists ? sub_off[c + 1] - sub_off[c] : 0ull;
#pragma unroll
            for (int o = 32; o >= 1; o >>= 1) ad += __shfl_xor(ad, o, 64);
            admitted += ad;
        }
    }
    if (lane == 0) rough_count[b] = sub_off ? admitted : carry;
    if (lane == 0 && stream_len) stream_len[b] = carry;
}
__global__ __launch_bounds__(256) void pair_prefix_kernel(PairScalars *__restrict__ scal, uint32_t nq, uint32_t nprobe,
                                                          unsigned long long *__restrict__ rough_count) {
    const uint32_t b = blockIdx.x * 4 + (threadIdx.x >> 6);
    if (b < nq) pair_prefix_row(scal, b, nprobe, rough_count);
}
__global__ __launch_bounds__(256) void pair_prefix_filtered_kernel(PairScalars *__restrict__ scal, uint32_t nq, uint32_t nprobe,
                                                                   unsigned long long *__restrict__ rough_count,
                                                                   const uint32_t *__restrict__ pair_cluster,
                                                                   const uint32_t *__restrict__ sub_off, uint32_t nlists,
                                                                   unsigned long long *__restrict__ stream_len) {
    const uint32_t b = blockIdx.x * 4 + (threadIdx.x >> 6);
    if (b < nq) pair_prefix_row(scal, b, nprobe, rough_count, pair_cluster, sub_off, nlists, stream_len);
}

__global__ __launch_bounds__(256) void filter_positions_kernel(const uint32_t *__restrict__ map_ids, uint64_t n,
                                                               const uint32_t *__restrict__ allow_ids, uint64_t nbits,
                                                               uint32_t *__restrict__ pos_bits, uint64_t nwords) {
    const uint64_t pos = (uint64_t)blockIdx.x * 256 + threadIdx.x;
    const uint32_t lane = threadIdx.x & 63;
    bool in = false;
    if (pos < n) {
        const uint32_t id = map_ids[pos];
        in = (uint64_t)id < nbits && ((allow_ids[id >> 5] >> (id & 31u)) & 1u);
    }
    const uint64_t m = __ballot(in);
    const uint64_t w = (pos - lane) >> 5;
    if (lane < 2 && w + lane < nwords) pos_bits[w + lane] = (uint32_t)(m >> (32 * lane));
}
__global__ __launch_bounds__(256) void filter_lists_kernel(const uint32_t *__restrict__ pos_bits, const uint32_t *__restrict__ offsets,
                                                           uint32_t *__restrict__ list_adm) {
    __shared__ uint32_t s_cnt;
    const uint32_t c = blockIdx.x;
    const uint32_t b = offsets[c], e = offsets[c + 1];
    if (threadIdx.x == 0) s_cnt = 0;
    __syncthreads();
    uint32_t cnt = 0;
    if (e > b) {
        for (uint32_t w = (b >> 5) + threadIdx.x; w <= ((e - 1) >> 5); w += 256) {
            uint32_t bits = pos_bits[w];
            const uint32_t w0 = w << 5;
            if (w0 < b) bits &= ~0u << (b - w0);
            if (e - w0 < 32) bits &= (1u << (e - w0)) - 1u;
            cnt += (uint32_t)__popc(bits);
        }
    }
    if (cnt) atomicAdd(&s_cnt, cnt);
    __syncthreads();
    if (threadIdx.x == 0) list_adm[c] = s_cnt;
}

__device__ __forceinline__ bool pair_in_stage(const PairScalars &ps, uint32_t s_lo, uint32_t s_hi) {
    const uint64_t b = ps.stream_begin, e = b + ps.list_len;
    return ps.list_len != 0 && b < s_hi && e > s_lo;
}

__global__ void group_count_kernel(const PairScalars *__restrict__ scal,
                                   const uint32_t *__restrict__ probe_cluster, uint32_t count, uint32_t nprobe,
                                   uint32_t slot_hi, uint32_t s_lo, uint32_t s_hi, uint32_t *__restrict__ grp_cnt) {
    const uint32_t i = blockIdx.x * blockDim.x + threadIdx.x;
    if (i >= count) return;
    const uint32_t b = i / slot_hi, p = b * nprobe + (i - b * slot_hi);
    if (pair_in_stage(scal[p], s_lo, s_hi)) atomicAdd(&grp_cnt[probe_cluster[p]], 1u);
}

#define RQ_RANK_ITEMS 32768u
__global__ __launch_bounds__(1024) void group_rank_kernel(const PairScalars *__restrict__ scal,
                                                          const uint32_t *__restrict__ probe_cluster, uint32_t count,
                                                          uint32_t nprobe, uint32_t slot_hi, uint32_t s_lo, uint32_t s_hi,
                                                          uint32_t k, uint32_t *__restrict__ grp_cnt,
                                                          uint32_t *__restrict__ rank, uint32_t *__restrict__ blk_base) {
    extern __shared__ uint32_t rank_hist[];
    for (uint32_t c = threadIdx.x; c < k; c += 1024) rank_hist[c] = 0;
    __syncthreads();
    const uint32_t first = blockIdx.x * RQ_RANK_ITEMS;
    for (uint32_t j = threadIdx.x; j < RQ_RANK_ITEMS; j += 1024) {
        const uint32_t i = first + j;
        if (i >= count) break;
        const uint32_t b = i / slot_hi, p = b * nprobe + (i - b * slot_hi);
        uint32_t r = ~0u;
        if (pair_in_stage(scal[p], s_lo, s_hi)) r = atomicAdd(&rank_hist[probe_cluster[p]], 1u);
        rank[i] = r;
    }
    __syncthreads();
    for (uint32_t c = threadIdx.x; c < k; c += 1024) {
        const uint32_t h = rank_hist[c];
        blk_base[(uint64_t)blockIdx.x * k + c] = h ? atomicAdd(&grp_cnt[c], h) : 0u;
    }
}

__global__ __launch_bounds__(1024) void group_scan_kernel(uint32_t *__restrict__ cnt, uint32_t k,
                                                          uint32_t *__restrict__ start, uint32_t pad32,
                                                          uint32_t *__restrict__ recs, uint32_t opdw) {
    __shared__ uint32_t wsum[16];
    __shared__ uint32_t carry;
    const uint32_t tid = threadIdx.x, lane = tid & 63, wid = tid >> 6;
    if (tid == 0) carry = 0;
    __syncthreads();
    for (uint32_t base = 0; base < k; base += 1024) {
        uint32_t i = base + tid;
        uint32_t v = i < k ? cnt[i] : 0;
        if (pad32 & 1u) v = (v + 31u) & ~31u;
        uint32_t incl = v;
        for (int o = 1; o < 64; o <<= 1) {
            uint32_t up = __shfl_up(incl, o, 64);
            if ((int)lane >= o) incl += up;
        }
        if (lane == 63) wsum[wid] = incl;
        __syncthreads();
        uint32_t woff = 0;
        for (uint32_t w = 0; w < wid; ++w) woff += wsum[w];
        uint32_t c0 = carry;
        if (i < k) {
            const uint32_t st0 = c0 + woff + incl - v;
            start[i] = st0;
            if ((pad32 & 1u) && recs) {
                const uint32_t real = cnt[i];
                const bool additive = (pad32 & 4u) != 0;
                const uint32_t opld = rq_img_opld(opdw, additive), img = rq_img_dwords(opdw, additive);
                for (uint32_t at = st0 + real; at < st0 + v; ++at) {
                    if (additive) {
                        recs[(uint64_t)(at >> 5) * img + 32 * opld + 32 * RQ_RECA_TAIL + (at & 31u)] = 0xFF800000u;
                        continue;
                    }
                    uint32_t *tl = recs + (uint64_t)(at >> 5) * img + 32 * opld + (at & 31u) * RQ_REC_TAIL + RQ_REC_V0;
                    *reinterpret_cast<uint4 *>(tl) = make_uint4(0u, 0u, 0u, 0x0000FF80u);
                    *reinterpret_cast<uint4 *>(tl + 4) = make_uint4(0u, 0u, 0u, 0u);
                }
            }
            if (!(pad32 & 2u)) cnt[i] = 0;
        }
        __syncthreads();
        if (tid == 1023) carry = c0 + woff + incl;
        __syncthreads();
    }
    if (tid == 0) start[k] = carry;
}

__device__ __forceinline__ uint32_t bf16_rne(float x) {
    uint32_t u = __builtin_bit_cast(uint32_t, x);
    u += 0x7FFFu + ((u >> 16) & 1u);
    return u >> 16;
}
__device__ __forceinline__ float bf16_to_f32(uint32_t b) { return __builtin_bit_cast(float, b << 16); }

template <int LPP = 16 >
__device__ __forceinline__ void stage_fill_item(const PairScalars *__restrict__ scal,
                                                const uint32_t *__restrict__ probe_cluster,
                                                const uint32_t *__restrict__ operand ,
                                                const float *__restrict__ thr, uint32_t wi,
                                                uint32_t nprobe, uint32_t slot_hi, uint32_t opdw, uint32_t s_lo,
                                                uint32_t s_hi,
                                                uint32_t cluster_major,
                                                const uint32_t *__restrict__ grp_start,
                                                uint32_t *__restrict__ grp_cursor,
                                                uint32_t *__restrict__ recs, const FactorStats &fs,
                                                uint32_t tile_images ,
                                                const uint32_t *__restrict__ rank ,
                                                const uint32_t *__restrict__ blk_base, uint32_t k,
                                                const float4 *__restrict__ list_uref ) {
    const uint32_t sub = threadIdx.x & (LPP - 1);
    if (cluster_major && rank && rank[wi] == ~0u) return;
    const uint32_t wb = wi / slot_hi, p = wb * nprobe + (wi - wb * slot_hi);
    const PairScalars ps = scal[p];
    const bool in = pair_in_stage(ps, s_lo, s_hi);
    if (cluster_major && !in) return;
    uint32_t at = p;
    uint32_t list_id = 0;
    if (cluster_major) {
        const uint32_t c = probe_cluster[p];
        list_id = c;
        if (rank) {
            at = grp_start[c] + blk_base[(uint64_t)(wi / RQ_RANK_ITEMS) * k + c] + rank[wi];
        } else {
            uint32_t a = 0;
            if (sub == 0) a = atomicAdd(&grp_cursor[c], 1u);
            at = grp_start[c] + __shfl(a, 0, LPP);
        }
    }
    const uint32_t stride = opdw + RQ_REC_TAIL;
    uint32_t *r = recs + (uint64_t)at * stride;
    uint32_t *tdst = r + opdw;
    float *cdst = nullptr;
    if (tile_images) {
        const uint32_t opld = rq_img_opld(opdw, tile_images == 2), img = rq_img_dwords(opdw, tile_images == 2);
        const uint32_t taild = tile_images == 2 ? RQ_RECA_TAIL : RQ_REC_TAIL;
        uint32_t *base = recs + (uint64_t)(at >> 5) * img;
        r = base + (at & 31u) * opld;
        tdst = base + 32 * opld + (at & 31u) * taild;
        if (tile_images == 2) cdst = reinterpret_cast<float *>(base + 32 * opld + 32 * taild + (at & 31u));
    }
    if constexpr (LPP == 8) {
        const uint4 *src = reinterpret_cast<const uint4 *>(operand + (uint64_t)p * opdw);
        uint4 *dst = reinterpret_cast<uint4 *>(r);
        for (uint32_t i = sub; i < opdw / 4; i += 8) dst[i] = src[i];
    } else {
        const uint2 *src = reinterpret_cast<const uint2 *>(operand + (uint64_t)p * opdw);
        uint2 *dst = reinterpret_cast<uint2 *>(r);
        for (uint32_t i = sub; i < opdw / 2; i += 16) dst[i] = src[i];
    }
    {
        uint32_t t[RQ_REC_TAIL];
        uint32_t lo = 0, hi = 0;
        if (in) {
            lo = s_lo > ps.stream_begin ? s_lo - ps.stream_begin : 0u;
            hi = s_hi - ps.stream_begin;
            hi = hi < ps.list_len ? hi : ps.list_len;
        }
        t[RQ_REC_LOWER] = __builtin_bit_cast(uint32_t, ps.lower);
        t[RQ_REC_DELTA] = __builtin_bit_cast(uint32_t, ps.delta);
        t[RQ_REC_SUMQ] = __builtin_bit_cast(uint32_t, ps.sumq);
        t[RQ_REC_YCD] = __builtin_bit_cast(uint32_t, ps.ycd);
        t[RQ_REC_YCD_SQRT] = __builtin_bit_cast(uint32_t, ps.ycd_sqrt);
        t[RQ_REC_THR] = __builtin_bit_cast(uint32_t, thr[ps.row]);
        t[RQ_REC_LO] = lo;
        t[RQ_REC_HI] = hi;
        t[RQ_REC_ROW] = ps.row;
        t[RQ_REC_SLOT] = p - ps.row * nprobe;
        t[RQ_REC_LIST_BEGIN] = ps.list_begin;
        t[RQ_REC_LIST_LEN] = ps.list_len;
        const float th = thr[ps.row];
        const float inv2d = 0.5f / ps.delta;
        float v[4] = {(th - ps.ycd) * inv2d, -inv2d, -ps.lower * inv2d, ps.ycd_sqrt * inv2d};
        const float qb = (fabsf(th - ps.ycd) + fs.cds_max + fabsf(ps.lower) * fs.ppc_absmax + ps.ycd_sqrt * fs.eb_max) *
                         fs.invfip_absmax * fabsf(inv2d);
        const bool safe = ps.delta > 0.0f && qb + ps.sumq < 524288.0f;
        const float margin = 2.0f + qb * (1.0f / 8192.0f) + (qb + ps.sumq) * (1.0f / 262144.0f);
        if (tile_images == 2) {
            const float4 u0 = list_uref[list_id];
            float bq = u0.x * v[0];
            bq += u0.y * v[1];
            bq += u0.w * v[3];
            bq += 0.5f * ps.sumq;
            const float margin_a = 2.0f + qb * (1.0f / 8192.0f) + (qb + ps.sumq) * (1.0f / 65536.0f);
            float cq = -0.5f * (bq - margin_a);
            if (!safe || !(fabsf(cq) < 1.0e37f)) cq = __builtin_inff();
            if (sub == 5) *cdst = cq;
            if (sub < 3) *reinterpret_cast<uint4 *>(tdst + 4 * sub) = make_uint4(t[4 * sub], t[4 * sub + 1], t[4 * sub + 2], t[4 * sub + 3]);
            return;
        }
        const float v4 = -0.5f * (0.5f * ps.sumq - margin);
        uint32_t vh[4], vl[4];
#pragma unroll
        for (int i = 0; i < 4; ++i) {
            const float x = -0.5f * v[i];
            vh[i] = bf16_rne(x);
            vl[i] = bf16_rne(x - bf16_to_f32(vh[i]));
        }
        uint32_t c0 = bf16_rne(v4);
        const float r1 = v4 - bf16_to_f32(c0);
        uint32_t c1 = bf16_rne(r1);
        uint32_t c2 = bf16_rne(r1 - bf16_to_f32(c1));
        if (!safe) {
#pragma unroll
            for (int i = 0; i < 4; ++i) vh[i] = 0, vl[i] = 0;
            c0 = 0x7F80u, c1 = 0, c2 = 0;
        }
        t[RQ_REC_V0 + 0] = vh[0] | (vh[0] << 16);
        t[RQ_REC_V0 + 1] = vl[0] | (vh[1] << 16);
        t[RQ_REC_V0 + 2] = vh[1] | (vl[1] << 16);
        t[RQ_REC_V0 + 3] = c0 | (c1 << 16);
        t[RQ_REC_V0 + 4] = vh[2] | (vh[2] << 16);
        t[RQ_REC_V0 + 5] = vl[2] | (vh[3] << 16);
        t[RQ_REC_V0 + 6] = vh[3] | (vl[3] << 16);
        t[RQ_REC_V0 + 7] = c2;
        if (!tile_images) t[RQ_REC_CELL0] = (ps.stream_begin >> 6) + 2u * (p - ps.row * nprobe) + 1u - (s_lo >> 6);
        static_assert(RQ_REC_TAIL == 20, "five 16-byte pieces");
        uint4 piece = make_uint4(t[0], t[1], t[2], t[3]);
#pragma unroll
        for (int i = 1; i < 5; ++i)
            if (sub == (uint32_t)i) piece = make_uint4(t[4 * i], t[4 * i + 1], t[4 * i + 2], t[4 * i + 3]);
        if (sub < 5) *reinterpret_cast<uint4 *>(tdst + 4 * sub) = piece;
    }
}
template <int LPP = 16>
__global__ __launch_bounds__(256) void stage_fill_kernel(const PairScalars *__restrict__ scal,
                                                         const uint32_t *__restrict__ probe_cluster,
                                                         const uint32_t *__restrict__ operand ,
                                                         const float *__restrict__ thr, uint32_t count,
                                                         uint32_t nprobe, uint32_t slot_hi, uint32_t opdw, uint32_t s_lo,
                                                         uint32_t s_hi,
                                                         uint32_t cluster_major,
                                                         const uint32_t *__restrict__ grp_start,
                                                         uint32_t *__restrict__ grp_cursor,
                                                         uint32_t *__restrict__ recs, const FactorStats fs,
                                                         uint32_t tile_images,
                                                         const uint32_t *__restrict__ rank ,
                                                         const uint32_t *__restrict__ blk_base, uint32_t k,
                                                         const float4 *__restrict__ list_uref,
                                                         const uint32_t *__restrict__ items = nullptr ) {
    uint32_t wi = blockIdx.x * (256 / LPP) + threadIdx.x / LPP;
    if (wi >= count) return;
    if (items) wi = items[wi];
    stage_fill_item<LPP>(scal, probe_cluster, operand, thr, wi, nprobe, slot_hi, opdw, s_lo, s_hi, cluster_major, grp_start, grp_cursor,
                    recs, fs, tile_images, rank, blk_base, k, list_uref);
}

__global__ __launch_bounds__(256) void group_vrange_kernel(const uint32_t *__restrict__ recs, const uint32_t *__restrict__ grp_start,
                                                           const uint32_t *__restrict__ grp_cnt, uint32_t opdw,
                                                           float4 *__restrict__ vref) {
    const uint32_t c = blockIdx.x, n = grp_cnt[c], st0 = grp_start[c];
    const uint32_t opld = rq_img_opld(opdw, true), img = rq_img_dwords(opdw, true);
    const float inf = __builtin_inff();
    float lo[4] = {inf, inf, inf, inf}, hi[4] = {-inf, -inf, -inf, -inf};
    for (uint32_t i = threadIdx.x; i < n; i += 256) {
        const uint32_t at = st0 + i;
        const uint32_t *base = recs + (uint64_t)(at >> 5) * img + 32 * opld;
        const float cq = __builtin_bit_cast(float, base[32 * RQ_RECA_TAIL + (at & 31u)]);
        if (!(cq < inf)) continue;
        const uint32_t *t = base + (at & 31u) * RQ_RECA_TAIL;
        const float lower = __builtin_bit_cast(float, t[RQ_REC_LOWER]), delta = __builtin_bit_cast(float, t[RQ_REC_DELTA]);
        const float ycd = __builtin_bit_cast(float, t[RQ_REC_YCD]), ysq = __builtin_bit_cast(float, t[RQ_REC_YCD_SQRT]);
        const float th = __builtin_bit_cast(float, t[RQ_REC_THR]);
        const float inv2d = 0.5f / delta;
        const float v[4] = {(th - ycd) * inv2d, -inv2d, -lower * inv2d, ysq * inv2d};
#pragma unroll
        for (int r = 0; r < 4; ++r) lo[r] = fminf(lo[r], v[r]), hi[r] = fmaxf(hi[r], v[r]);
    }
    __shared__ float red[4][8];
#pragma unroll
    for (int r = 0; r < 4; ++r) {
        for (int o = 32; o >= 1; o >>= 1) lo[r] = fminf(lo[r], __shfl_xor(lo[r], o, 64)), hi[r] = fmaxf(hi[r], __shfl_xor(hi[r], o, 64));
    }
    if ((threadIdx.x & 63) == 0) {
#pragma unroll
        for (int r = 0; r < 4; ++r) red[threadIdx.x >> 6][r] = lo[r], red[threadIdx.x >> 6][4 + r] = hi[r];
    }
    __syncthreads();
    if (threadIdx.x == 0) {
        float v0[4], dv[4];
#pragma unroll
        for (int r = 0; r < 4; ++r) {
            const float l = fminf(fminf(red[0][r], red[1][r]), fminf(red[2][r], red[3][r]));
            const float u = fmaxf(fmaxf(red[0][4 + r], red[1][4 + r]), fmaxf(red[2][4 + r], red[3][4 + r]));
            const bool any = l <= u && u < inf && l > -inf;
            v0[r] = any ? 0.5f * l + 0.5f * u : 0.0f;
            dv[r] = any ? fmaxf(u - v0[r], v0[r] - l) * 1.000001f : 0.0f;
        }
        vref[2 * c] = make_float4(v0[0], v0[1], v0[2], v0[3]);
        vref[2 * c + 1] = make_float4(dv[0], dv[1], dv[2], dv[3]);
    }
}


template <bool FILT>
__device__ __forceinline__ void scan_generic_body(SCAN_PARAMS, uint32_t W) {
    const uint32_t STRIDE = 8 * W + RQ_REC_TAIL;
    const uint32_t gl = blockIdx.x / a.tiles_per_group;
    const uint32_t g = a.group_base + gl;
    const uint32_t tile = a.tile_base + (blockIdx.x - gl * a.tiles_per_group);
    uint32_t pb, pe;
    if (a.cluster_major) {
        pb = grp_start[g];
        pe = grp_start[g + 1];
    } else {
        pb = g;
        pe = g + 1;
    }
    if (pb >= pe) return;
    const uint32_t lane = threadIdx.x & 63;
    const uint32_t wave = __builtin_amdgcn_readfirstlane(threadIdx.x >> 6);
    const uint32_t *rec = recs + (uint64_t)pb * STRIDE;
    const uint32_t list_begin = rec[8 * W + RQ_REC_LIST_BEGIN], list_len = rec[8 * W + RQ_REC_LIST_LEN];
    const uint32_t first = tile * 256;
    if (first >= list_len) return;
    if (!a.cluster_major && rec[8 * W + RQ_REC_LO] >= rec[8 * W + RQ_REC_HI]) return;
    const uint32_t local = first + threadIdx.x;
    const uint32_t pos = list_begin + (local < list_len ? local : 0);
    const uint32_t *cp = codes + (uint64_t)pos * (2 * W);
    const float4 fac = factors[pos];
    bool adm = true;
    if constexpr (FILT) {
        adm = rq_admitted(load_scan_extra(a.x).allow, pos) != 0u;
        if (!__syncthreads_or(adm)) return;
    }
    for (uint32_t i = pb; i < pe; ++i, rec += STRIDE) {
        const uint32_t *pl = rec;
        const uint32_t *t = rec + 8 * W;
        const uint32_t lo_p = t[RQ_REC_LO], hi_p = t[RQ_REC_HI];
        if (hi_p <= first || lo_p >= first + 256) continue;
        uint32_t s = 0;
        for (int pp = 0; pp < 4; ++pp) {
            uint32_t tt = 0;
            for (uint32_t w = 0; w < 2 * W; ++w) tt += __popc(cp[w] & pl[pp * 2 * W + w]);
            s += tt << pp;
        }
        float rough = rough_distance(s, fac, __builtin_bit_cast(float, t[RQ_REC_LOWER]),
                                     __builtin_bit_cast(float, t[RQ_REC_DELTA]), __builtin_bit_cast(float, t[RQ_REC_SUMQ]),
                                     __builtin_bit_cast(float, t[RQ_REC_YCD]), __builtin_bit_cast(float, t[RQ_REC_YCD_SQRT]));
        const uint32_t P0 = first + wave * 64;
        const uint32_t ra = lo_p > P0 ? (lo_p - P0 < 64 ? lo_p - P0 : 64) : 0;
        const uint32_t rb = hi_p > P0 ? (hi_p - P0 < 64 ? hi_p - P0 : 64) : 0;
        const uint64_t below_b = rb >= 64 ? ~0ull : ((1ull << rb) - 1ull);
        const uint64_t below_a = ra >= 64 ? ~0ull : ((1ull << ra) - 1ull);
        uint64_t m = __ballot(rough < __builtin_bit_cast(float, t[RQ_REC_THR]) && adm) & below_b & ~below_a;
        if (m) {
            const uint32_t b = t[RQ_REC_ROW], slot = t[RQ_REC_SLOT];
            const bool pass = (m >> lane) & 1ull;
            const uint32_t cntc = (uint32_t)__popcll(m);
            unsigned long long old = 0;
            if (lane == 0) old = atomicAdd(surv_cnt + b, (1ull << 32) | cntc);
            uint32_t base = __builtin_amdgcn_readfirstlane((uint32_t)old);
            uint32_t rbase = __builtin_amdgcn_readfirstlane((uint32_t)(old >> 32));
            if (pass) {
                uint32_t at = base + (uint32_t)__popcll(m & ((1ull << lane) - 1ull));
                if (at < scan_seg(a).capof(b)) {
                    SurvRec r;
                    r.pos = pos, r.slot = slot, r.rough = rough, r.accurate = 0.0f;
                    surv[scan_seg(a).at(b) + at] = r;
                }
            }
            if (lane == 0 && rbase < scan_seg(a).capof(b)) {
                RunRec rr;
                rr.pos = list_begin + first + (threadIdx.x & ~63u);
                rr.slot = slot, rr.base = base, rr.cnt = cntc;
                runs[scan_seg(a).at(b) + rbase] = rr;
            }
        }
    }
}
__global__ __launch_bounds__(256) void scan_generic_kernel(SCAN_PARAMS, uint32_t W) {
    scan_generic_body<false>(codes, factors, offsets, grp_start, recs, surv, runs, surv_cnt, tile_table, a, W);
}
__global__ __launch_bounds__(256) void scan_generic_filtered_kernel(SCAN_PARAMS, uint32_t W) {
    scan_generic_body<true>(codes, factors, offsets, grp_start, recs, surv, runs, surv_cnt, tile_table, a, W);
}

__global__ __launch_bounds__(256) void scan_dense_kernel(const uint32_t *__restrict__ codes,
                                                         const float4 *__restrict__ factors,
                                                         uint32_t list_begin, uint32_t list_len,
                                                         uint32_t W, const uint32_t *__restrict__ pl,
                                                         float lower, float delta, float sumq, float ycd,
                                                         float *__restrict__ out) {
    uint32_t i = blockIdx.x * 256 + threadIdx.x;
    if (i >= list_len) return;
    const uint32_t *cp = codes + (uint64_t)(list_begin + i) * (2 * W);
    uint32_t s = 0;
    for (int p = 0; p < 4; ++p) {
        uint32_t t = 0;
        for (uint32_t w = 0; w < 2 * W; ++w) t += __popc(cp[w] & pl[p * 2 * W + w]);
        s += t << p;
    }
    out[i] = rough_distance(s, factors[list_begin + i], lower, delta, sumq, ycd, sqrtf(ycd));
}

__global__ __launch_bounds__(256) void accurate_flat_kernel(const uint32_t *__restrict__ pos, uint32_t m,
                                                            const BaseView base,
                                                            const float *__restrict__ q, uint32_t dim,
                                                            float *__restrict__ out) {
    const uint32_t l = threadIdx.x & 7;
    uint32_t i = blockIdx.x * 32 + (threadIdx.x >> 3);
    if (i >= m) return;
    const RowRef x = base.row(pos[i], dim);
    float acc = 0.0f;
    for (uint32_t c = 0; c < dim; c += 8) {
        float d = rq_row_get(x, dim, c + l) - q[c + l];
        acc = fmaf(d, d, acc);
    }
    acc = reduce8_lanes(acc);
    if (l == 0) out[i] = acc;
}

#define RQ_SORT_LDS_RECS 2048
template <typename T, uint32_t LDS_RECS = RQ_SORT_LDS_RECS>
__device__ __forceinline__ void sort_segment(T *recs, uint32_t n, const T *src = nullptr ) {
    __shared__ T lds[LDS_RECS];
    if (!src) src = recs;
    if (n < 2 && src == recs) return;
    auto key = [](const T &r) { return surv_key(r); };
    if (n <= LDS_RECS) {
        for (uint32_t i = threadIdx.x; i < n; i += blockDim.x) lds[i] = src[i];
        __syncthreads();
        bitonic_sort_block(lds, n, key);
        for (uint32_t i = threadIdx.x; i < n; i += blockDim.x) recs[i] = lds[i];
    } else {
        if (src != recs) {
            for (uint32_t i = threadIdx.x; i < n; i += blockDim.x) recs[i] = src[i];
            __threadfence_block();
        }
        __syncthreads();
        bitonic_sort_block(recs, n, key);
    }
}
#define RQ_BUCKET_CHUNK 1024u
#define RQ_SORT_MID_LDS_WORDS 14336u
template <uint32_t MAX_SLOTS>
__device__ __forceinline__ void sort_runs_by_slot(RunRec *__restrict__ dir, RunRec *__restrict__ tmp, uint32_t n, uint32_t nslots) {
    __shared__ uint32_t start[MAX_SLOTS + 1], cursor[MAX_SLOTS];
    __shared__ uint32_t wsum[16];
    __shared__ __attribute__((aligned(16))) uint32_t keys[4][RQ_BUCKET_CHUNK];
    const uint32_t tid = threadIdx.x, nthr = blockDim.x, lane = tid & 63, wave = tid >> 6, nwaves = nthr >> 6;
    for (uint32_t i = tid; i < nslots; i += nthr) cursor[i] = 0;
    __syncthreads();
    for (uint32_t i = tid; i < n; i += nthr) atomicAdd(&cursor[dir[i].slot], 1u);
    __syncthreads();
    {
// ... 1246 lines not shown
```

### rabitq_amd/csrc/rabitq_hip.hip

```cpp
#include "../../include/rabitq_hip.h"

#include <hip/hip_runtime.h>

#include <algorithm>
#include <charconv>
#include <chrono>
#include <atomic>
#include <cmath>
#include <cstdio>
#include <cstdlib>
#include <cstring>
#include <memory>
#include <mutex>
#include <random>
#include <string>
#include <thread>
#include <vector>
#include <sys/stat.h>
#include <dlfcn.h>
#include <queue>
#include <map>

#include "common.h"
#include "kernels_build.h"
// ... 616 lines not shown
    return RQ_OK;
}
rq_status rq_filter_rows(const rq_filter *f, uint64_t *out_admitted) {
    if (!f || !out_admitted) return fail(RQ_ERR_INVALID, "null argument");
    *out_admitted = f->rows;
    return RQ_OK;
}
void rq_filter_free(rq_filter *f) { delete f; }

static rq_status mutate_done(const rq_index *idx, rq_status s, std::chrono::steady_clock::time_point t0) {
    if (s != RQ_OK) (void)hipGetLastError();
    if (idx) g_mutate_stats.rows_after = idx->n;
    g_mutate_stats.ms_total = std::chrono::duration<float, std::milli>(std::chrono::steady_clock::now() - t0).count();
    return s;
}
rq_status rq_add(rq_index *idx, const float *rows, uint64_t m, uint32_t d, const uint32_t *ids, int rows_on_device,
                 uint32_t *out_first_id) {
    const auto t0 = std::chrono::steady_clock::now();
    return mutate_done(idx, index_add(idx, rows, m, d, ids, rows_on_device, out_first_id), t0);
}
rq_status rq_remove(rq_index *idx, const uint32_t *id_bits, uint64_t nbits, int bits_on_device, uint64_t *out_removed) {
    const auto t0 = std::chrono::steady_clock::now();
    return mutate_done(idx, index_remove(idx, id_bits, nbits, bits_on_device, out_removed), t0);
}
rq_status rq_last_mutate_stats(rq_mutate_stats_t *out) {
    if (!out) return fail(RQ_ERR_INVALID, "null argument");
    return copy_out_sized(out, g_mutate_stats);
}

rq_status rq_query(const rq_index *idx, const float *query, uint32_t len, uint32_t probe, uint32_t topk,
                   int heuristic_rank, float *out_dist, uint32_t *out_id, uint32_t *out_n) {
    return rq_query_batch(idx, query, 1, len, probe, topk, heuristic_rank, out_dist, out_id, out_n);
}

#include "host_shard.h"

rq_status rq_metrics(rq_metrics_t *out) {
    if (!out) return fail(RQ_ERR_INVALID, "null argument");
    out->rough = g_rough.load(), out->precise = g_precise.load(), out->query = g_query.load(), out->miss = g_miss.load();
    return RQ_OK;
}
rq_status rq_metrics_reset(void) {
    g_rough = 0, g_precise = 0, g_query = 0, g_miss = 0;
    return RQ_OK;
}

rq_status rq_set_option(const char *name, int value) {
    if (!name) return fail(RQ_ERR_INVALID, "null option name");
    if (std::string(name) == "scan_impl") {
        if (value < 0 || value > 2) return fail(RQ_ERR_INVALID, "scan_impl must be 0 (auto), 1 (valu) or 2 (mfma)");
        g_scan_impl = value;
        return RQ_OK;
    }
    if (std::string(name) == "cluster_major_div") {
        if (value < 1 || value > 4096) return fail(RQ_ERR_INVALID, "cluster_major_div must be in [1, 4096]");
        g_cluster_major_div = value;
        return RQ_OK;
    }
    if (std::string(name) == "large_batch_from") {
        if (value < 2 || value > (1 << 20)) return fail(RQ_ERR_INVALID, "large_batch_from must be in [2, 2^20]");
        g_large_from = value;
        return RQ_OK;
    }
    if (std::string(name) == "stage_settle_pct") {
        if (value < 1 || value > 400) return fail(RQ_ERR_INVALID, "stage_settle_pct must be in [1, 400]");
        g_stage_settle_pct = value;
        return RQ_OK;
    }
    if (std::string(name) == "stage_growth") {
        if (value != 0 && (value < 2 || value > 64)) return fail(RQ_ERR_INVALID, "stage_growth must be 0 or in [2, 64]");
        g_stage_growth = value;
        return RQ_OK;
    }
    if (std::string(name) == "base_device_mb") {
        if (value < -1) return fail(RQ_ERR_INVALID, "base_device_mb must be >= -1");
        g_base_device_mb = value;
        return RQ_OK;
    }
    if (std::string(name) == "pass_overlap") {
        if (value < 0 || value > 1) return fail(RQ_ERR_INVALID, "pass_overlap must be 0 or 1");
        g_pass_overlap = value;
        return RQ_OK;
    }
    if (std::string(name) == "split_rows") {
        if (value < 0 || value > 2) return fail(RQ_ERR_INVALID, "split_rows must be 0, 1 or 2");
        g_split_rows = value;
        return RQ_OK;
    }
    if (std::string(name) == "scan_tile_table") {
        if (value < 0 || value > 2) return fail(RQ_ERR_INVALID, "scan_tile_table must be 0 (never), 1 (auto) or 2 (always)");
        g_scan_tile_table = value;
        return RQ_OK;
    }
    if (std::string(name) == "max_scan_blocks") {
        if (value < 0) return fail(RQ_ERR_INVALID, "max_scan_blocks must be >= 0");
        g_max_scan_blocks = value == 0 ? RQ_MAX_BLOCKS_256 : std::min<uint32_t>((uint32_t)value, RQ_MAX_BLOCKS_256);
        return RQ_OK;
    }
    if (std::string(name) == "pair_split") {
        if (value < 0 || value > 1) return fail(RQ_ERR_INVALID, "pair_split must be 0 or 1");
        g_pair_split = value;
        return RQ_OK;
    }
    if (std::string(name) == "coarse_tiled_from") {
        if (value < 0) return fail(RQ_ERR_INVALID, "coarse_tiled_from must be >= 0");
        g_coarse_tiled_from = value;
        return RQ_OK;
    }
    if (std::string(name) == "coarse_impl") {
        if (value < 0 || value > 4) return fail(RQ_ERR_INVALID, "coarse_impl must be 0, 1, 2, 3 or 4");
        g_coarse_impl = value;
        return RQ_OK;
    }
    if (std::string(name) == "survivor_segments") {
#ifdef RQ_DEV_ABLATIONS
        if (value < 0 || value > 3) return fail(RQ_ERR_INVALID, "survivor_segments must be 0, 1, 2 or 3");
#else
        if (value == 3) return fail(RQ_ERR_INVALID, "survivor_segments = 3 (allocation-failure injection) exists in the developer build only (make dev)");
        if (value < 0 || value > 2) return fail(RQ_ERR_INVALID, "survivor_segments must be 0, 1 or 2");
#endif
        g_seg_opt = value;
        return RQ_OK;
    }
    if (std::string(name) == "assign_impl") {
        if (value < 0 || value > 1) return fail(RQ_ERR_INVALID, "assign_impl must be 0 or 1");
        g_assign_impl = value;
        return RQ_OK;
    }
    if (std::string(name) == "small_batch_span") {
        if (value < 1) return fail(RQ_ERR_INVALID, "small_batch_span must be >= 1");
        g_sb_span = value;
        return RQ_OK;
    }
    if (std::string(name) == "small_batch") {
        if (value < 0 || value > 1) return fail(RQ_ERR_INVALID, "small_batch must be 0 or 1");
        g_small_batch = value;
        return RQ_OK;
    }
    if (std::string(name) == "dense_dir") {
        if (value < 0 || value > 1) return fail(RQ_ERR_INVALID, "dense_dir must be 0 or 1");
        g_dense_dir = value;
        return RQ_OK;
    }
    if (std::string(name) == "shared_thresholds") {
        if (value < 0 || value > 2) return fail(RQ_ERR_INVALID, "shared_thresholds must be 0, 1 or 2");
        g_shared_thr = value;
        return RQ_OK;
    }
    if (std::string(name) == "group_rank") {
        if (value < 0 || value > 2) return fail(RQ_ERR_INVALID, "group_rank must be 0, 1 or 2");
        g_group_rank = value;
        return RQ_OK;
    }
    if (std::string(name) == "rerank_shadow") {
        if (value < 0 || value > 2) return fail(RQ_ERR_INVALID, "rerank_shadow must be 0 (never), 1 (fp16 rows when they fit) or 2 (8-bit rows when they fit)");
        g_rerank_shadow = value;
        return RQ_OK;
    }
    if (std::string(name) == "scan_gate") {
        if (value < 0 || value > 2) return fail(RQ_ERR_INVALID, "scan_gate must be 0, 1 or 2");
        g_scan_gate = value;
        return RQ_OK;
    }
    if (std::string(name) == "scan_debug") {
#ifdef RQ_DEV_ABLATIONS
        const int allowed = 0x7FFFFFFF;
#else
        const int allowed = 128 | 512 | 4096 | 16384;
#endif
        if (value < 0 || (value & ~allowed)) return fail(RQ_ERR_INVALID, "scan_debug: this bit exists in the developer build only (librabitq_hip_dev.so)");
        g_scan_dbg = value;
        return RQ_OK;
    }
    return fail(RQ_ERR_INVALID, std::string("unknown option ") + name);
}

rq_status rq_set_profiling(int level) {
    if (level < 0 || level > 2) return fail(RQ_ERR_INVALID, "profiling level must be 0, 1 or 2");
    g_profiling = level;
    return RQ_OK;
}
rq_status rq_last_profile(rq_profile_t *out) {
    if (!out) return fail(RQ_ERR_INVALID, "null argument");
    return copy_out_sized(out, g_profile);
}

rq_status rq_rotate(const float *x, uint64_t n, uint32_t dim, const float *orthogonal, int use_mfma, float *out) {
    RQC(ensure_device());
    if (!x || !orthogonal || !out) return fail(RQ_ERR_INVALID, "null argument");
    if (dim == 0 || dim % 64) return fail(RQ_ERR_DIM_MISMATCH, "dim must be a multiple of 64");
    DevBuf<float> dx, dp, dout;
    RQC(dx.alloc(n * dim));
    RQC(dp.alloc((size_t)dim * dim));
    RQC(dout.alloc(n * dim));
    HIPC(hipMemcpy(dx.p, x, n * dim * 4, hipMemcpyHostToDevice));
    HIPC(hipMemcpy(dp.p, orthogonal, (size_t)dim * dim * 4, hipMemcpyHostToDevice));
    launch_rotate(dx.p, dp.p, dout.p, n, dim, use_mfma != 0, nullptr);
    HIPC(hipDeviceSynchronize());
    HIPC(hipGetLastError());
    HIPC(hipMemcpy(out, dout.p, n * dim * 4, hipMemcpyDeviceToHost));
    return RQ_OK;
}

rq_status rq_rotate_device(const rq_index *idx, const float *d_x, uint64_t n, float *d_out, float *out_ms) {
    RQC(ensure_device());
    if (!idx || !d_x || !d_out) return fail(RQ_ERR_INVALID, "null argument");
    hipEvent_t e0, e1;
    HIPC(hipEventCreate(&e0));
    HIPC(hipEventCreate(&e1));
    HIPC(hipEventRecord(e0, nullptr));
    launch_rotate(d_x, idx->P.p, d_out, n, idx->dim, true, nullptr);
    HIPC(hipEventRecord(e1, nullptr));
    HIPC(hipEventSynchronize(e1));
    HIPC(hipGetLastError());
    float ms = 0;
    HIPC(hipEventElapsedTime(&ms, e0, e1));
    if (out_ms) *out_ms = ms;
    (void)hipEventDestroy(e0);
    (void)hipEventDestroy(e1);
    return RQ_OK;
}

rq_status rq_quantize_pack(const float *x_rot, uint64_t n, uint32_t dim, const float *centroids_rot, uint32_t k,
                           uint32_t *out_label, float *out_dist, uint64_t *out_codes, rq_factor_t *out_factors) {
    RQC(ensure_device());
    RQC(ensure_kernel_attributes());
    if (!x_rot || !centroids_rot || !out_label || !out_dist || !out_codes || !out_factors)
        return fail(RQ_ERR_INVALID, "null argument");
    if (dim == 0 || dim % 64 || k == 0) return fail(RQ_ERR_DIM_MISMATCH, "dim must be a multiple of 64, k > 0");
    rq_index tmp;
    tmp.dim = dim, tmp.k = k, tmp.W = dim / 64;
    DevBuf<float> dx, dd;
    DevBuf<uint32_t> dl;
    DevBuf<uint64_t> dc;
    DevBuf<float4> df;
    RQC(dx.alloc(n * dim));
    RQC(tmp.centroids.alloc((size_t)k * dim));
    RQC(tmp.cent_t.alloc((size_t)k * dim));
    RQC(dd.alloc(n));
    RQC(dl.alloc(n));
    RQC(dc.alloc(n * tmp.W));
    RQC(df.alloc(n));
    HIPC(hipMemcpy(dx.p, x_rot, n * dim * 4, hipMemcpyHostToDevice));
    HIPC(hipMemcpy(tmp.centroids.p, centroids_rot, (size_t)k * dim * 4, hipMemcpyHostToDevice));
    transpose_kernel<<<dim3(ceil_div(dim, 32), ceil_div(k, 32)), dim3(32, 8)>>>(tmp.centroids.p, tmp.cent_t.p, k, dim);
    AssignAux ax;
    HIPC(hipDeviceSynchronize());
    if (assign_has_mfma(tmp.W) && g_assign_impl.load() != 1) RQC(assign_aux_init(&tmp, ax, std::min<uint64_t>(std::max<uint64_t>(n, 1), 1ull << 20)));
    for (uint64_t i0 = 0; i0 < n; i0 += (1ull << 20)) {
        const uint64_t m = std::min<uint64_t>(1ull << 20, n - i0);
        RQC(launch_assign_prefiltered(dx.p + i0 * dim, &tmp, ax, m, dl.p + i0, dd.p + i0));
        quantize_kernel<<<ceil_div(m, 32), 256>>>(dx.p + i0 * dim, tmp.centroids.p, dl.p + i0, m, dim,
                                                  dc.p + i0 * tmp.W, df.p + i0);
    }
    HIPC(hipDeviceSynchronize());
    HIPC(hipGetLastError());
    if (n) {
        HIPC(hipMemcpy(out_label, dl.p, n * 4, hipMemcpyDeviceToHost));
        HIPC(hipMemcpy(out_dist, dd.p, n * 4, hipMemcpyDeviceToHost));
        HIPC(hipMemcpy(out_codes, dc.p, n * tmp.W * 8, hipMemcpyDeviceToHost));
        HIPC(hipMemcpy(out_factors, df.p, n * 16, hipMemcpyDeviceToHost));
    }
    return RQ_OK;
}

rq_status rq_coarse_rank(const rq_index *idx, const float *queries, uint32_t nq, uint32_t len, uint32_t probe,
                         float *out_y, uint32_t *out_cluster, float *out_dist) {
    RQC(ensure_device());
    if (!idx || !queries || !out_cluster || !out_dist) return fail(RQ_ERR_INVALID, "null argument");
    if (idx->dim != (len + 63) / 64 * 64) return fail(RQ_ERR_DIM_MISMATCH, "query length does not pad to dim");
    if (probe == 0) return fail(RQ_ERR_INVALID, "probe == 0");
    const uint32_t dim = idx->dim, k = idx->k, nprobe = std::min(probe, k);
    if (nprobe > RQ_MAX_PROBE) return fail(RQ_ERR_UNSUPPORTED, "probe > 16384");
    DevBuf<float> dq, qpad, y, dist, pd;
    DevBuf<uint32_t> pc;
    RQC(dq.alloc((uint64_t)nq * len));
    RQC(qpad.alloc((uint64_t)nq * dim));
    RQC(y.alloc((uint64_t)nq * dim));
    RQC(dist.alloc((uint64_t)nq * k));
    RQC(pd.alloc((uint64_t)nq * nprobe));
    RQC(pc.alloc((uint64_t)nq * nprobe));
    HIPC(hipMemcpy(dq.p, queries, (uint64_t)nq * len * 4, hipMemcpyHostToDevice));
    pad_rows_kernel<<<ceil_div((uint64_t)nq * dim, 256), 256>>>(dq.p, qpad.p, nq, len, dim);
    launch_rotate(qpad.p, idx->P.p, y.p, nq, dim, nq >= 32, nullptr);
    coarse_dist_kernel<4><<<dim3(ceil_div(nq, 4), ceil_div(k, 256)), 256, 4 * dim * sizeof(float)>>>(
        idx->cent_t.p, y.p, dist.p, k, dim, nq, k);
    launch_select(dist.p, k, nprobe, pc.p, pd.p, 0, nprobe, nq, nullptr);
    HIPC(hipDeviceSynchronize());
    HIPC(hipGetLastError());
    if (out_y) HIPC(hipMemcpy(out_y, y.p, (uint64_t)nq * dim * 4, hipMemcpyDeviceToHost));
    HIPC(hipMemcpy(out_cluster, pc.p, (uint64_t)nq * nprobe * 4, hipMemcpyDeviceToHost));
    HIPC(hipMemcpy(out_dist, pd.p, (uint64_t)nq * nprobe * 4, hipMemcpyDeviceToHost));
    return RQ_OK;
}

rq_status rq_query_prep(const rq_index *idx, const float *y, uint32_t nq, const uint32_t *cluster, float *out_lower,
                        float *out_delta, uint32_t *out_sum, uint64_t *out_planes) {
    RQC(ensure_device());
    if (!idx || !y || !cluster || !out_lower || !out_delta || !out_sum || !out_planes)
        return fail(RQ_ERR_INVALID, "null argument");
    const uint32_t dim = idx->dim, W = idx->W;
    for (uint32_t i = 0; i < nq; ++i)
        if (cluster[i] >= idx->k) return fail(RQ_ERR_INVALID, "cluster id out of range");
    DevBuf<float> dy, ycd;
    DevBuf<uint32_t> dc, dsum;
    DevBuf<PairScalars> scal;
// ... 68 lines not shown
```

Measured before the change: 3.820 million.

## Place final-stage fp6 query records directly into cluster-grouped tile images during prep

When the last stage runs on the matrix path, the group ranking for that stage is computed before quantisation. The prep kernel then writes each pair's fp6 operand row and tail straight into its final cluster-major tile image slot, instead of writing qf6 rows that a later fill kernel regroups. A small stage_tail kernel fills in thresholds and gate coefficients in place, and several memsets are folded into one clear kernel. The aim is to remove a full extra pass of writing and re-reading the per-pair operand records. The cost is extra ranking work up front and a larger preallocated image buffer.

New measurement: 3.916 million, median of 6. 1.03x the previous value.

```diff
diff --git a/rabitq_amd/csrc/host_query.h b/rabitq_amd/csrc/host_query.h
--- a/rabitq_amd/csrc/host_query.h
+++ b/rabitq_amd/csrc/host_query.h
@@ -197,6 +197,8 @@
     bool sb_results_done = false;
     bool sb_fused_finish = false;
     bool sb_filled = false;
+    bool placed = false;
+    bool fin_additive = false;
     if (small) {
         const int gopt = g_stage_growth.load();
         stages = build_stages(16ull * std::max<uint32_t>(topk, 1), gopt >= 2 ? (uint64_t)gopt : 8, (uint64_t)std::max(1, g_sb_span.load()));
@@ -293,6 +295,43 @@
         const uint64_t growth = gopt >= 2 ? (uint64_t)gopt : (nq >= 32768 ? 8 : 16);
         stages = build_stages((uint64_t)std::max<uint32_t>(topk, 1) * (rq_large_batch(nq) ? growth : 1), growth, ~0ull);
     }
+    const bool prep_dim = dim == 64 || dim == 128 || dim == 256 || dim == 512 || dim == 768 || dim == 1024;
+    const bool will_list = (filt || (idx->nonempty_lists * 2 < k && npairs >= 65536)) && g_pair_split.load() != 0 && prep_dim;
+    if (g_prep_placement.load() != 0 && !filt && !ext_cluster && !d_row_map && !qp.thr_init && !qp.seg_final && !will_list && prep_dim &&
+        scan_is_fused(W) && k <= 32768 && !stages.empty() && stages.back().s_hi == 0xFFFFFFFFu && stage_on_matrix(stages.back())) {
+        placed = true;
+        for (size_t i = 0; i + 1 < stages.size(); ++i) placed = placed && !stage_on_matrix(stages[i]);
+        const int rank_opt = g_group_rank.load();
+        placed = placed && (rank_opt == 2 || (rank_opt == 1 && npairs >= 16 * RQ_RANK_ITEMS && npairs / RQ_RANK_ITEMS >= k / 256));
+        const int gate_opt = g_scan_gate.load();
+        fin_additive = scan_has_additive(W) && idx->list_uref.p != nullptr && gate_opt != 1 && (gate_opt == 2 || !idx->additive_loose.load());
+    }
+    if (placed) {
+        const Stage &fin = stages.back();
+        const uint32_t nblk = ceil_div(npairs, RQ_RANK_ITEMS);
+        RQC(ws.img_final.ensure(((size_t)npairs + 32ull * k + 32) * (12ull * W + 2 + RQ_REC_TAIL)));
+        RQC(ws.pair_begin.ensure(npairs));
+        RQC(ws.fin_rank.ensure(npairs));
+        RQC(ws.fin_rank_base.ensure((size_t)nblk * k));
+        RQC(ws.fin_grp_cnt.ensure(k + 4));
+        RQC(ws.fin_grp_start.ensure(k + 1));
+        if (fin_additive) RQC(ws.grp_vref.ensure(2 * (size_t)k));
+        pf.begin(PF_GROUP);
+        {
+            ClearSpans cs{};
+            cs.p[0] = reinterpret_cast<uint32_t *>(ws.totals.p), cs.n[0] = 16;
+            cs.p[1] = reinterpret_cast<uint32_t *>(ws.stat.p), cs.n[1] = 512;
+            cs.p[2] = ws.big_list.p + nq, cs.n[2] = 3;
+            cs.p[3] = ws.fin_grp_cnt.p, cs.n[3] = k + 4;
+            if (rq_large_batch(nq)) cs.p[4] = ws.q_hist.p, cs.n[4] = k + 2;
+            clear_words_kernel<<<std::max(2u, ceil_div(k + 4, 256)), 256, 0, st>>>(cs);
+        }
+        pair_prefix_lens_kernel<<<ceil_div(nq, 4), 256, 0, st>>>(idx->offsets.p, probe_cluster, k, nq, nprobe, ws.rough_cnt.p, ws.pair_begin.p, ws.scal.p);
+        group_rank_kernel<<<nblk, 1024, (size_t)k * 4, st>>>(nullptr, probe_cluster, npairs, nprobe, nprobe, fin.s_lo, fin.s_hi, k, ws.fin_grp_cnt.p,
+                                                            ws.fin_rank.p, ws.fin_rank_base.p, ws.pair_begin.p, idx->offsets.p);
+        group_scan_kernel<<<1, 1024, 0, st>>>(ws.fin_grp_cnt.p, k, ws.fin_grp_start.p, 1u | 2u | (fin_additive ? 4u : 0u), ws.img_final.p, 12 * W);
+        pf.end();
+    }
     pf.begin(PF_PREP);
     {
         uint32_t *qn = scan_is_fused(W) ? ws.qnib.p : nullptr;
@@ -318,9 +357,17 @@
             HIPC(hipStreamSynchronize(st));
             nlive = (uint32_t)*h_live;
         }
+        PrepPlace pl{};
+        if (placed) {
+            pl.stream_begin = ws.pair_begin.p, pl.rank = ws.fin_rank.p, pl.blk_base = ws.fin_rank_base.p, pl.grp_start = ws.fin_grp_start.p;
+            pl.img = ws.img_final.p, pl.s_lo = stages.back().s_lo, pl.s_hi = stages.back().s_hi, pl.tile_images = fin_additive ? 2u : 1u;
+        }
 #define RQ_PREP_SMALL(LP, R, PPB, PP)                                                                              \
     do {                                                                                                           \
-        if (listed)                                                                                                \
+        if (placed)                                                                                                \
+            prep_small_placed_kernel<LP, R, PP><<<ceil_div(npairs, (PPB) * (PP)), 256, 0, st>>>(ws.y.p, idx->centroids.p, idx->offsets.p, probe_cluster, \
+                                                                    probe_dist, npairs, nprobe, ws.scal.p, qn, k, idx->nonempty_lists * 2 < k ? 2u : 1u, qn_slots, pl); \
+        else if (listed)                                                                                           \
             prep_small_listed_kernel<LP, R, PP><<<std::max(1u, ceil_div(nlive, (PPB) * (PP))), 256, 0, st>>>(ws.y.p, idx->centroids.p, idx->offsets.p, probe_cluster, \
                                                                     probe_dist, ws.live_list.p, nlive, nprobe, ws.scal.p, qn, q6, k); \
         else                                                                                                       \
@@ -344,10 +391,10 @@
         RQC(ws.stream_len.ensure(nq));
         pair_prefix_filtered_kernel<<<ceil_div(nq, 4), 256, 0, st>>>(ws.scal.p, nq, nprobe, ws.rough_cnt.p, probe_cluster, filt->sub_off.p, k,
                                                                      ws.stream_len.p);
-    } else
+    } else if (!placed)
         pair_prefix_kernel<<<ceil_div(nq, 4), 256, 0, st>>>(ws.scal.p, nq, nprobe, ws.rough_cnt.p);
     if (rq_large_batch(nq)) {
-        HIPC(hipMemsetAsync(ws.q_hist.p, 0, (size_t)(k + 2) * 4, st));
+        if (!placed) HIPC(hipMemsetAsync(ws.q_hist.p, 0, (size_t)(k + 2) * 4, st));
         order_count_kernel<<<ceil_div(nq, 256), 256, 0, st>>>(probe_cluster, nprobe, nq, k, ws.q_hist.p);
         group_scan_kernel<<<1, 1024, 0, st>>>(ws.q_hist.p, k + 1, ws.q_start.p, 0u, nullptr, 0u);
         order_scatter_kernel<<<ceil_div(nq, 256), 256, 0, st>>>(probe_cluster, nprobe, nq, k, ws.q_start.p, ws.q_hist.p,
@@ -355,9 +402,11 @@
         rerank_order = ws.q_order.p;
     }
     init_state_kernel<<<ceil_div(nq, 256), 256, 0, st>>>(rs, ws.surv_cnt.p, nq, qp.thr_init, d_row_map);
-    HIPC(hipMemsetAsync(ws.totals.p, 0, 8 * sizeof(unsigned long long), st));
-    HIPC(hipMemsetAsync(ws.big_list.p + nq, 0, 12, st));
-    HIPC(hipMemsetAsync(ws.stat.p, 0, 256 * sizeof(unsigned long long), st));
+    if (!placed) {
+        HIPC(hipMemsetAsync(ws.totals.p, 0, 8 * sizeof(unsigned long long), st));
+        HIPC(hipMemsetAsync(ws.big_list.p + nq, 0, 12, st));
+        HIPC(hipMemsetAsync(ws.stat.p, 0, 256 * sizeof(unsigned long long), st));
+    }
     pf.end();
 
     }
@@ -381,8 +430,12 @@
         const bool fp6_records = use_mfma;
         const bool arena_stage = qp.seg_final && span > qp.cap && scan_is_fused(W) && rq_large_batch(nq);
         const int gate_opt = g_scan_gate.load();
-        const bool additive = use_mfma && !arena_stage && !filt && scan_has_additive(W) && idx->list_uref.p != nullptr && gate_opt != 1 &&
-                              (gate_opt == 2 || !idx->additive_loose.load());
+        const bool placed_stage = placed && stage_no + 1 == stages.size();
+        if (placed_stage && (g_scan_dbg.load() & 16384))
+            fprintf(stderr, "[rabitq_hip] stage %u: placed ahead of the quantisation (%s gate)\n", stage_no, fin_additive ? "additive" : "bf16");
+        const bool additive = placed_stage ? fin_additive
+                                           : use_mfma && !arena_stage && !filt && scan_has_additive(W) && idx->list_uref.p != nullptr && gate_opt != 1 &&
+                                                 (gate_opt == 2 || !idx->additive_loose.load());
         pf.begin(PF_GROUP);
         ScanArgs a{};
         ScanPtrs sp{};
@@ -392,7 +445,12 @@
             slot_hi = (uint32_t)std::min<uint64_t>(nprobe, (uint64_t)(sg.s_hi - 1) / min_len + 1);
         const uint32_t stage_pairs = nq * slot_hi;
         bool ranked = false;
-        if (cluster_major) {
+        if (placed_stage) {
+            stage_tail_kernel<<<k, 256, 0, st>>>(ws.img_final.p, ws.fin_grp_start.p, ws.fin_grp_cnt.p, ws.thr.p, 12 * W, idx->fstats,
+                                                 additive ? 2u : 1u, idx->list_uref.p, ws.grp_vref.p);
+            if (additive) ws.pend_additive = true;
+            a.ngroups = k;
+        } else if (cluster_major) {
             HIPC(hipMemsetAsync(ws.grp_cnt.p, 0, (size_t)((k + 4) & ~3u) * 4, st));
             const int rank_opt = g_group_rank.load();
             ranked = k <= 32768 && (rank_opt == 2 || (rank_opt == 1 && stage_pairs >= 16 * RQ_RANK_ITEMS &&
@@ -413,7 +471,7 @@
         }
         const uint32_t *operand = fp6_records ? ws.qf6.p
                                               : (scan_is_fused(W) ? ws.qnib.p : reinterpret_cast<const uint32_t *>(ws.planes.p));
-        if (!(sb_filled && !cluster_major)) {
+        if (!(sb_filled && !cluster_major) && !placed_stage) {
             const bool fill_listed = listed && ranked && cluster_major && slot_hi == nprobe;
             const uint32_t fill_items = fill_listed ? nlive : stage_pairs;
             const bool fill8 = !use_mfma || additive;
@@ -432,7 +490,7 @@
                                                                     ws.rank_base.p, k, idx->list_uref.p, fill_listed ? ws.live_list.p : nullptr);
             }
         }
-        if (additive) {
+        if (additive && !placed_stage) {
             RQC(ws.grp_vref.ensure(2 * (size_t)k));
             group_vrange_kernel<<<k, 256, 0, st>>>(ws.recs.p, ws.grp_start.p, ws.grp_cnt.p, 12 * W, ws.grp_vref.p);
             ws.pend_additive = true;
@@ -440,10 +498,10 @@
         pf.end();
         sp.codes = reinterpret_cast<const uint32_t *>(idx->codes.p);
         sp.factors = idx->factors.p;
-        sp.grp_start = ws.grp_start.p;
-        sp.grp_cnt = ws.grp_cnt.p;
+        sp.grp_start = placed_stage ? ws.fin_grp_start.p : ws.grp_start.p;
+        sp.grp_cnt = placed_stage ? ws.fin_grp_cnt.p : ws.grp_cnt.p;
         sp.offsets = idx->offsets.p;
-        sp.recs = ws.recs.p;
+        sp.recs = placed_stage ? ws.img_final.p : ws.recs.p;
         sp.surv = ws.surv.p;
         sp.runs = ws.runs.p;
         sp.surv_cnt = ws.surv_cnt.p;
diff --git a/rabitq_amd/csrc/host_state.h b/rabitq_amd/csrc/host_state.h
--- a/rabitq_amd/csrc/host_state.h
+++ b/rabitq_amd/csrc/host_state.h
@@ -170,6 +170,7 @@
     DevBuf<uint32_t> live_list;
     DevBuf<uint32_t> coarse_redo;
     DevBuf<uint32_t> pair_rank, rank_base;
+    DevBuf<uint32_t> img_final, pair_begin, fin_rank, fin_rank_base, fin_grp_cnt, fin_grp_start;
     DevBuf<uint32_t> probe_cluster, recs, grp_cnt, grp_start, heap_len, heap_id, precise, need,
         nsurv, nshadow, win_count, arr_len, row_map, big_list;
     DevBuf<int32_t> heap_key;
@@ -533,6 +534,7 @@
 static std::atomic<int> g_cluster_major_div{32};
 static std::atomic<int> g_stage_settle_pct{100};
 static std::atomic<int> g_scan_tile_table{1};
+static std::atomic<int> g_prep_placement{1};
 static std::atomic<int> g_group_rank{1};
 static std::atomic<int> g_shared_thr{1};
 static std::atomic<int> g_sb_span{2560};
diff --git a/rabitq_amd/csrc/kernels_query.h b/rabitq_amd/csrc/kernels_query.h
--- a/rabitq_amd/csrc/kernels_query.h
+++ b/rabitq_amd/csrc/kernels_query.h
@@ -870,7 +870,38 @@
     }
 }
 
-template <int LP, int R, int PP>
+__device__ __forceinline__ bool stream_in_stage(uint32_t begin, uint32_t len, uint32_t s_lo, uint32_t s_hi) {
+    const uint64_t b = begin, e = b + len;
+    return len != 0 && b < s_hi && e > s_lo;
+}
+#define RQ_RANK_ITEMS 32768u
+__device__ __forceinline__ void stage_tail_static(const PairScalars &ps, bool in, uint32_t slot, uint32_t s_lo, uint32_t s_hi,
+                                                  uint32_t *__restrict__ t) {
+    uint32_t lo = 0, hi = 0;
+    if (in) {
+        lo = s_lo > ps.stream_begin ? s_lo - ps.stream_begin : 0u;
+        hi = s_hi - ps.stream_begin;
+        hi = hi < ps.list_len ? hi : ps.list_len;
+    }
+    t[RQ_REC_LOWER] = __builtin_bit_cast(uint32_t, ps.lower);
+    t[RQ_REC_DELTA] = __builtin_bit_cast(uint32_t, ps.delta);
+    t[RQ_REC_SUMQ] = __builtin_bit_cast(uint32_t, ps.sumq);
+    t[RQ_REC_YCD] = __builtin_bit_cast(uint32_t, ps.ycd);
+    t[RQ_REC_YCD_SQRT] = __builtin_bit_cast(uint32_t, ps.ycd_sqrt);
+    t[RQ_REC_LO] = lo;
+    t[RQ_REC_HI] = hi;
+    t[RQ_REC_ROW] = ps.row;
+    t[RQ_REC_SLOT] = slot;
+    t[RQ_REC_LIST_BEGIN] = ps.list_begin;
+    t[RQ_REC_LIST_LEN] = ps.list_len;
+}
+struct PrepPlace {
+    const uint32_t *stream_begin;
+    const uint32_t *rank, *blk_base, *grp_start;
+    uint32_t *img;
+    uint32_t s_lo, s_hi, tile_images;
+};
+template <int LP, int R, int PP, bool PLACE = false>
 __device__ __forceinline__ void prep_small_pairs(const float *__restrict__ y, const float *__restrict__ centroids,
                                                  const uint32_t *__restrict__ offsets,
                                                  const uint32_t *__restrict__ pair_cluster,
@@ -879,7 +910,8 @@
                                                  uint32_t *__restrict__ qnib, uint32_t *__restrict__ qf6,
                                                  uint32_t nlists, uint32_t skip_empty, uint32_t p0,
                                                  const uint32_t *__restrict__ live_list = nullptr ,
-                                                 uint32_t qn_slots = 0xFFFFFFFFu ) {
+                                                 uint32_t qn_slots = 0xFFFFFFFFu ,
+                                                 const PrepPlace &pl = PrepPlace{} ) {
     static_assert(R >= 1 && (LP == 16 || LP == 32 || LP == 64), "lane groups of 16 / 32 / 64; a round = 4 LP dimensions (the packing's neighbour exchanges stay inside a round)");
     constexpr uint32_t DIM = 4 * LP * R, W = DIM / 64, PPW = 64 / LP;
     const uint32_t lane = threadIdx.x & 63, sub = lane % LP;
@@ -887,6 +919,7 @@
     float ycd_in[PP];
     bool live[PP];
     uint32_t pid[PP];
+    uint32_t sbeg[PP], place[PP];
 #pragma unroll
     for (int pp = 0; pp < PP; ++pp) {
         const uint32_t pi = p0 + pp * PPW;
@@ -895,6 +928,11 @@
         const uint32_t p = pid[pp];
         cl[pp] = live[pp] ? pair_cluster[p] : 0xFFFFFFFFu;
         ycd_in[pp] = live[pp] ? pair_ycd[p] : 0.0f;
+        sbeg[pp] = 0u, place[pp] = ~0u;
+        if constexpr (PLACE) {
+            sbeg[pp] = live[pp] ? pl.stream_begin[p] : 0u;
+            place[pp] = live[pp] ? pl.rank[p] : ~0u;
+        }
     }
     float4 cv[PP][R], yv[PP][R];
 #pragma unroll
@@ -903,6 +941,10 @@
         const bool in = live[pp] && c < nlists;
         lb[pp] = in ? offsets[c] : 0u;
         ll[pp] = in ? offsets[c + 1] - lb[pp] : 0u;
+        if constexpr (PLACE) {
+            if (in && place[pp] != ~0u) place[pp] += pl.grp_start[c] + pl.blk_base[(uint64_t)(p / RQ_RANK_ITEMS) * nlists + c];
+            else place[pp] = ~0u;
+        }
         const uint32_t row = live[pp] ? p / pairs_per_row : 0u;
         const bool fetch = skip_empty == 2 ? ll[pp] != 0 : true;
 #pragma unroll
@@ -924,10 +966,22 @@
             if (sub == 0) {
                 PairScalars s;
                 s.lower = 0.0f, s.delta = 0.0f, s.sumq = 0.0f, s.ycd = ycd_in[pp], s.ycd_sqrt = 0.0f;
-                s.row = row, s.list_begin = 0, s.list_len = 0, s.stream_begin = 0, s.pad = 0;
+                s.row = row, s.list_begin = 0, s.list_len = 0, s.stream_begin = sbeg[pp], s.pad = 0;
                 scal[p] = s;
             }
             continue;
+        }
+        uint32_t *q6row = qf6 ? qf6 + (uint64_t)p * 12 * W : nullptr;
+        uint32_t *tail_dst = nullptr;
+        if constexpr (PLACE) {
+            q6row = nullptr;
+            if (place[pp] != ~0u) {
+                const bool additive = pl.tile_images == 2;
+                const uint32_t opld = rq_img_opld(12 * W, additive), at = place[pp];
+                uint32_t *base = pl.img + (uint64_t)(at >> 5) * rq_img_dwords(12 * W, additive);
+                q6row = base + (at & 31u) * opld;
+                tail_dst = base + 32 * opld + (at & 31u) * (additive ? RQ_RECA_TAIL : RQ_REC_TAIL);
+            }
         }
         float r[R][4];
         float mn = 3.402823466e+38f, mx = -3.402823466e+38f;
@@ -970,9 +1024,9 @@
             {
                 const uint32_t nxt = __shfl_down(f24, 1, LP);
                 const uint32_t t = dsub & 7, sh = 8 * (t & 3);
-                if (qf6 && (t & 3) != 3) {
+                if (q6row && (t & 3) != 3) {
                     const uint32_t w = dsub >> 4, h = (dsub >> 3) & 1;
-                    qf6[(uint64_t)p * 12 * W + h * 6 * W + 6 * w + 3 * (t >> 2) + (t & 3)] = (f24 >> sh) | (nxt << (24 - sh));
+                    q6row[h * 6 * W + 6 * w + 3 * (t >> 2) + (t & 3)] = (f24 >> sh) | (nxt << (24 - sh));
                 }
             }
         }
@@ -988,9 +1042,18 @@
             s.row = row;
             s.list_begin = lb[pp];
             s.list_len = ll[pp];
-            s.stream_begin = 0;
+            s.stream_begin = sbeg[pp];
             s.pad = 0;
             scal[p] = s;
+            if constexpr (PLACE) {
+                if (tail_dst) {
+                    uint32_t t[12];
+                    stage_tail_static(s, true, p - row * pairs_per_row, pl.s_lo, pl.s_hi, t);
+                    t[RQ_REC_THR] = 0u;
+#pragma unroll
+                    for (int i = 0; i < 3; ++i) reinterpret_cast<uint4 *>(tail_dst)[i] = make_uint4(t[4 * i], t[4 * i + 1], t[4 * i + 2], t[4 * i + 3]);
+                }
+            }
         }
     }
 }
@@ -1010,6 +1073,21 @@
                                 skip_empty, p0, nullptr, qn_slots);
 }
 
+template <int LP, int R, int PP>
+__global__ __launch_bounds__(256) void prep_small_placed_kernel(const float *__restrict__ y,
+                                                                const float *__restrict__ centroids,
+                                                                const uint32_t *__restrict__ offsets,
+                                                                const uint32_t *__restrict__ pair_cluster,
+                                                                const float *__restrict__ pair_ycd, uint32_t npairs,
+                                                                uint32_t pairs_per_row, PairScalars *__restrict__ scal,
+                                                                uint32_t *__restrict__ qnib, uint32_t nlists,
+                                                                uint32_t skip_empty, uint32_t qn_slots, const PrepPlace pl) {
+    constexpr uint32_t PPW = 64 / LP;
+    const uint32_t p0 = (blockIdx.x * 4 + (threadIdx.x >> 6)) * (PPW * PP) + (threadIdx.x & 63) / LP;
+    prep_small_pairs<LP, R, PP, true>(y, centroids, offsets, pair_cluster, pair_ycd, npairs, pairs_per_row, scal, qnib, nullptr, nlists,
+                                      skip_empty, p0, nullptr, qn_slots, pl);
+}
+
 __global__ __launch_bounds__(1024) void pair_split_kernel(const uint32_t *__restrict__ offsets, const uint32_t *__restrict__ pair_cluster,
                                                           const float *__restrict__ pair_ycd, uint32_t npairs, uint32_t pairs_per_row,
                                                           uint32_t nlists, PairScalars *__restrict__ scal,
@@ -1072,13 +1150,20 @@
                                                 unsigned long long *__restrict__ rough_count,
                                                 const uint32_t *__restrict__ pair_cluster = nullptr,
                                                 const uint32_t *__restrict__ sub_off = nullptr, uint32_t nlists = 0,
-                                                unsigned long long *__restrict__ stream_len = nullptr) {
+                                                unsigned long long *__restrict__ stream_len = nullptr,
+                                                const uint32_t *__restrict__ offsets = nullptr ,
+                                                uint32_t *__restrict__ begin_out = nullptr ) {
     const uint32_t lane = threadIdx.x & 63;
     unsigned long long carry = 0, admitted = 0;
     for (uint32_t s0 = 0; s0 < nprobe; s0 += 64) {
         const uint32_t s = s0 + lane;
         PairScalars *ps = scal + (uint64_t)b * nprobe + s;
-        const unsigned long long len = s < nprobe ? ps->list_len : 0;
+        unsigned long long len = 0;
+        if (offsets) {
+            const uint32_t c = s < nprobe ? pair_cluster[(uint64_t)b * nprobe + s] : 0xFFFFFFFFu;
+            len = c < nlists ? offsets[c + 1] - offsets[c] : 0u;
+        } else
+            len = s < nprobe ? ps->list_len : 0;
         unsigned long long incl = len;
 #pragma unroll
         for (int o = 1; o < 64; o <<= 1) {
@@ -1086,7 +1171,7 @@
             if ((int)lane >= o) incl += up;
         }
         const unsigned long long begin = carry + incl - len;
-        if (s < nprobe) ps->stream_begin = begin > 0xFFFFFFFFull ? 0xFFFFFFFFu : (uint32_t)begin;
+        if (s < nprobe) *(begin_out ? begin_out + (uint64_t)b * nprobe + s : &ps->stream_begin) = begin > 0xFFFFFFFFull ? 0xFFFFFFFFu : (uint32_t)begin;
         carry += __shfl(incl, 63, 64);
         if (sub_off) {
             const uint32_t c = s < nprobe && len ? pair_cluster[(uint64_t)b * nprobe + s] : 0xFFFFFFFFu;
@@ -1103,6 +1188,13 @@
                                                           unsigned long long *__restrict__ rough_count) {
     const uint32_t b = blockIdx.x * 4 + (threadIdx.x >> 6);
     if (b < nq) pair_prefix_row(scal, b, nprobe, rough_count);
+}
+__global__ __launch_bounds__(256) void pair_prefix_lens_kernel(const uint32_t *__restrict__ offsets, const uint32_t *__restrict__ pair_cluster,
+                                                               uint32_t nlists, uint32_t nq, uint32_t nprobe,
+                                                               unsigned long long *__restrict__ rough_count, uint32_t *__restrict__ begin_out,
+                                                               PairScalars *__restrict__ scal ) {
+    const uint32_t b = blockIdx.x * 4 + (threadIdx.x >> 6);
+    if (b < nq) pair_prefix_row(scal, b, nprobe, rough_count, pair_cluster, nullptr, nlists, nullptr, offsets, begin_out);
 }
 __global__ __launch_bounds__(256) void pair_prefix_filtered_kernel(PairScalars *__restrict__ scal, uint32_t nq, uint32_t nprobe,
                                                                    unsigned long long *__restrict__ rough_count,
@@ -1150,8 +1242,7 @@
 }
 
 __device__ __forceinline__ bool pair_in_stage(const PairScalars &ps, uint32_t s_lo, uint32_t s_hi) {
-    const uint64_t b = ps.stream_begin, e = b + ps.list_len;
-    return ps.list_len != 0 && b < s_hi && e > s_lo;
+    return stream_in_stage(ps.stream_begin, ps.list_len, s_lo, s_hi);
 }
 
 __global__ void group_count_kernel(const PairScalars *__restrict__ scal,
@@ -1163,12 +1254,13 @@
     if (pair_in_stage(scal[p], s_lo, s_hi)) atomicAdd(&grp_cnt[probe_cluster[p]], 1u);
 }
 
-#define RQ_RANK_ITEMS 32768u
 __global__ __launch_bounds__(1024) void group_rank_kernel(const PairScalars *__restrict__ scal,
                                                           const uint32_t *__restrict__ probe_cluster, uint32_t count,
                                                           uint32_t nprobe, uint32_t slot_hi, uint32_t s_lo, uint32_t s_hi,
                                                           uint32_t k, uint32_t *__restrict__ grp_cnt,
-                                                          uint32_t *__restrict__ rank, uint32_t *__restrict__ blk_base) {
+                                                          uint32_t *__restrict__ rank, uint32_t *__restrict__ blk_base,
+                                                          const uint32_t *__restrict__ begins = nullptr,
+                                                          const uint32_t *__restrict__ offsets = nullptr) {
     extern __shared__ uint32_t rank_hist[];
     for (uint32_t c = threadIdx.x; c < k; c += 1024) rank_hist[c] = 0;
     __syncthreads();
@@ -1178,7 +1270,11 @@
         if (i >= count) break;
         const uint32_t b = i / slot_hi, p = b * nprobe + (i - b * slot_hi);
         uint32_t r = ~0u;
-        if (pair_in_stage(scal[p], s_lo, s_hi)) r = atomicAdd(&rank_hist[probe_cluster[p]], 1u);
+        if (begins) {
+            const uint32_t c = probe_cluster[p];
+            if (c < k && stream_in_stage(begins[p], offsets[c + 1] - offsets[c], s_lo, s_hi)) r = atomicAdd(&rank_hist[c], 1u);
+        } else if (pair_in_stage(scal[p], s_lo, s_hi))
+            r = atomicAdd(&rank_hist[probe_cluster[p]], 1u);
         rank[i] = r;
     }
     __syncthreads();
@@ -1242,6 +1338,59 @@
     return u >> 16;
 }
 __device__ __forceinline__ float bf16_to_f32(uint32_t b) { return __builtin_bit_cast(float, b << 16); }
+
+struct StageGate {
+    float v[4], qb, margin;
+    bool safe;
+};
+__device__ __forceinline__ StageGate stage_gate(float lower, float delta, float sumq, float ycd, float ycd_sqrt, float th,
+                                                const FactorStats &fs) {
+    StageGate g;
+    const float inv2d = 0.5f / delta;
+    g.v[0] = (th - ycd) * inv2d, g.v[1] = -inv2d, g.v[2] = -lower * inv2d, g.v[3] = ycd_sqrt * inv2d;
+    g.qb = (fabsf(th - ycd) + fs.cds_max + fabsf(lower) * fs.ppc_absmax + ycd_sqrt * fs.eb_max) *
+           fs.invfip_absmax * fabsf(inv2d);
+    g.safe = delta > 0.0f && g.qb + sumq < 524288.0f;
+    g.margin = 2.0f + g.qb * (1.0f / 8192.0f) + (g.qb + sumq) * (1.0f / 262144.0f);
+    return g;
+}
+__device__ __forceinline__ float stage_gate_cq(const StageGate &g, float sumq, const float4 u0) {
+    float bq = u0.x * g.v[0];
+    bq += u0.y * g.v[1];
+    bq += u0.w * g.v[3];
+    bq += 0.5f * sumq;
+    const float margin_a = 2.0f + g.qb * (1.0f / 8192.0f) + (g.qb + sumq) * (1.0f / 65536.0f);
+    float cq = -0.5f * (bq - margin_a);
+    if (!g.safe || !(fabsf(cq) < 1.0e37f)) cq = __builtin_inff();
+    return cq;
+}
+__device__ __forceinline__ void stage_gate_bf16(const StageGate &g, float sumq, uint32_t *__restrict__ t8) {
+    const float v4 = -0.5f * (0.5f * sumq - g.margin);
+    uint32_t vh[4], vl[4];
+#pragma unroll
+    for (int i = 0; i < 4; ++i) {
+        const float x = -0.5f * g.v[i];
+        vh[i] = bf16_rne(x);
+        vl[i] = bf16_rne(x - bf16_to_f32(vh[i]));
+    }
+    uint32_t c0 = bf16_rne(v4);
+    const float r1 = v4 - bf16_to_f32(c0);
+    uint32_t c1 = bf16_rne(r1);
+    uint32_t c2 = bf16_rne(r1 - bf16_to_f32(c1));
+    if (!g.safe) {
+#pragma unroll
+        for (int i = 0; i < 4; ++i) vh[i] = 0, vl[i] = 0;
+        c0 = 0x7F80u, c1 = 0, c2 = 0;
+    }
+    t8[0] = vh[0] | (vh[0] << 16);
+    t8[1] = vl[0] | (vh[1] << 16);
+    t8[2] = vh[1] | (vl[1] << 16);
+    t8[3] = c0 | (c1 << 16);
+    t8[4] = vh[2] | (vh[2] << 16);
+    t8[5] = vl[2] | (vh[3] << 16);
+    t8[6] = vh[3] | (vl[3] << 16);
+    t8[7] = c2;
+}
 
 template <int LPP = 16 >
 __device__ __forceinline__ void stage_fill_item(const PairScalars *__restrict__ scal,
@@ -1300,69 +1449,16 @@
     }
     {
         uint32_t t[RQ_REC_TAIL];
-        uint32_t lo = 0, hi = 0;
-        if (in) {
-            lo = s_lo > ps.stream_begin ? s_lo - ps.stream_begin : 0u;
-            hi = s_hi - ps.stream_begin;
-            hi = hi < ps.list_len ? hi : ps.list_len;
-        }
-        t[RQ_REC_LOWER] = __builtin_bit_cast(uint32_t, ps.lower);
-        t[RQ_REC_DELTA] = __builtin_bit_cast(uint32_t, ps.delta);
-        t[RQ_REC_SUMQ] = __builtin_bit_cast(uint32_t, ps.sumq);
-        t[RQ_REC_YCD] = __builtin_bit_cast(uint32_t, ps.ycd);
-        t[RQ_REC_YCD_SQRT] = __builtin_bit_cast(uint32_t, ps.ycd_sqrt);
+        stage_tail_static(ps, in, p - ps.row * nprobe, s_lo, s_hi, t);
         t[RQ_REC_THR] = __builtin_bit_cast(uint32_t, thr[ps.row]);
-        t[RQ_REC_LO] = lo;
-        t[RQ_REC_HI] = hi;
-        t[RQ_REC_ROW] = ps.row;
-        t[RQ_REC_SLOT] = p - ps.row * nprobe;
-        t[RQ_REC_LIST_BEGIN] = ps.list_begin;
-        t[RQ_REC_LIST_LEN] = ps.list_len;
-        const float th = thr[ps.row];
-        const float inv2d = 0.5f / ps.delta;
-        float v[4] = {(th - ps.ycd) * inv2d, -inv2d, -ps.lower * inv2d, ps.ycd_sqrt * inv2d};
-        const float qb = (fabsf(th - ps.ycd) + fs.cds_max + fabsf(ps.lower) * fs.ppc_absmax + ps.ycd_sqrt * fs.eb_max) *
-                         fs.invfip_absmax * fabsf(inv2d);
-        const bool safe = ps.delta > 0.0f && qb + ps.sumq < 524288.0f;
-        const float margin = 2.0f + qb * (1.0f / 8192.0f) + (qb + ps.sumq) * (1.0f / 262144.0f);
+        const StageGate g = stage_gate(ps.lower, ps.delta, ps.sumq, ps.ycd, ps.ycd_sqrt, thr[ps.row], fs);
         if (tile_images == 2) {
-            const float4 u0 = list_uref[list_id];
-            float bq = u0.x * v[0];
-            bq += u0.y * v[1];
-            bq += u0.w * v[3];
-            bq += 0.5f * ps.sumq;
-            const float margin_a = 2.0f + qb * (1.0f / 8192.0f) + (qb + ps.sumq) * (1.0f / 65536.0f);
-            float cq = -0.5f * (bq - margin_a);
-            if (!safe || !(fabsf(cq) < 1.0e37f)) cq = __builtin_inff();
+            const float cq = stage_gate_cq(g, ps.sumq, list_uref[list_id]);
             if (sub == 5) *cdst = cq;
             if (sub < 3) *reinterpret_cast<uint4 *>(tdst + 4 * sub) = make_uint4(t[4 * sub], t[4 * sub + 1], t[4 * sub + 2], t[4 * sub + 3]);
             return;
         }
-        const float v4 = -0.5f * (0.5f * ps.sumq - margin);
-        uint32_t vh[4], vl[4];
-#pragma unroll
-        for (int i = 0; i < 4; ++i) {
-            const float x = -0.5f * v[i];
-            vh[i] = bf16_rne(x);
-            vl[i] = bf16_rne(x - bf16_to_f32(vh[i]));
-        }
-        uint32_t c0 = bf16_rne(v4);
-        const float r1 = v4 - bf16_to_f32(c0);
-        uint32_t c1 = bf16_rne(r1);
-        uint32_t c2 = bf16_rne(r1 - bf16_to_f32(c1));
-        if (!safe) {
-#pragma unroll
-            for (int i = 0; i < 4; ++i) vh[i] = 0, vl[i] = 0;
-            c0 = 0x7F80u, c1 = 0, c2 = 0;
-        }
-        t[RQ_REC_V0 + 0] = vh[0] | (vh[0] << 16);
-        t[RQ_REC_V0 + 1] = vl[0] | (vh[1] << 16);
-        t[RQ_REC_V0 + 2] = vh[1] | (vl[1] << 16);
-        t[RQ_REC_V0 + 3] = c0 | (c1 << 16);
-        t[RQ_REC_V0 + 4] = vh[2] | (vh[2] << 16);
-        t[RQ_REC_V0 + 5] = vl[2] | (vh[3] << 16);
-        t[RQ_REC_V0 + 6] = vh[3] | (vl[3] << 16);
-        t[RQ_REC_V0 + 7] = c2;
+        stage_gate_bf16(g, ps.sumq, t + RQ_REC_V0);
         if (!tile_images) t[RQ_REC_CELL0] = (ps.stream_begin >> 6) + 2u * (p - ps.row * nprobe) + 1u - (s_lo >> 6);
         static_assert(RQ_REC_TAIL == 20, "five 16-byte pieces");
         uint4 piece = make_uint4(t[0], t[1], t[2], t[3]);
@@ -1395,6 +1491,31 @@
                     recs, fs, tile_images, rank, blk_base, k, list_uref);
 }
 
+__device__ __forceinline__ void vrange_reduce_store(float *lo, float *hi, uint32_t c, float4 *__restrict__ vref, float (*red)[8] ) {
+    const float inf = __builtin_inff();
+#pragma unroll
+    for (int r = 0; r < 4; ++r) {
+        for (int o = 32; o >= 1; o >>= 1) lo[r] = fminf(lo[r], __shfl_xor(lo[r], o, 64)), hi[r] = fmaxf(hi[r], __shfl_xor(hi[r], o, 64));
+    }
+    if ((threadIdx.x & 63) == 0) {
+#pragma unroll
+        for (int r = 0; r < 4; ++r) red[threadIdx.x >> 6][r] = lo[r], red[threadIdx.x >> 6][4 + r] = hi[r];
+    }
+    __syncthreads();
+    if (threadIdx.x == 0) {
+        float v0[4], dv[4];
+#pragma unroll
+        for (int r = 0; r < 4; ++r) {
+            const float l = fminf(fminf(red[0][r], red[1][r]), fminf(red[2][r], red[3][r]));
+            const float u = fmaxf(fmaxf(red[0][4 + r], red[1][4 + r]), fmaxf(red[2][4 + r], red[3][4 + r]));
+            const bool any = l <= u && u < inf && l > -inf;
+            v0[r] = any ? 0.5f * l + 0.5f * u : 0.0f;
+            dv[r] = any ? fmaxf(u - v0[r], v0[r] - l) * 1.000001f : 0.0f;
+        }
+        vref[2 * c] = make_float4(v0[0], v0[1], v0[2], v0[3]);
+        vref[2 * c + 1] = make_float4(dv[0], dv[1], dv[2], dv[3]);
+    }
+}
 __global__ __launch_bounds__(256) void group_vrange_kernel(const uint32_t *__restrict__ recs, const uint32_t *__restrict__ grp_start,
                                                            const uint32_t *__restrict__ grp_cnt, uint32_t opdw,
                                                            float4 *__restrict__ vref) {
@@ -1417,30 +1538,60 @@
         for (int r = 0; r < 4; ++r) lo[r] = fminf(lo[r], v[r]), hi[r] = fmaxf(hi[r], v[r]);
     }
     __shared__ float red[4][8];
-#pragma unroll
-    for (int r = 0; r < 4; ++r) {
-        for (int o = 32; o >= 1; o >>= 1) lo[r] = fminf(lo[r], __shfl_xor(lo[r], o, 64)), hi[r] = fmaxf(hi[r], __shfl_xor(hi[r], o, 64));
-    }
-    if ((threadIdx.x & 63) == 0) {
-#pragma unroll
-        for (int r = 0; r < 4; ++r) red[threadIdx.x >> 6][r] = lo[r], red[threadIdx.x >> 6][4 + r] = hi[r];
-    }
-    __syncthreads();
-    if (threadIdx.x == 0) {
-        float v0[4], dv[4];
-#pragma unroll
-        for (int r = 0; r < 4; ++r) {
-            const float l = fminf(fminf(red[0][r], red[1][r]), fminf(red[2][r], red[3][r]));
-            const float u = fmaxf(fmaxf(red[0][4 + r], red[1][4 + r]), fmaxf(red[2][4 + r], red[3][4 + r]));
-            const bool any = l <= u && u < inf && l > -inf;
-            v0[r] = any ? 0.5f * l + 0.5f * u : 0.0f;
-            dv[r] = any ? fmaxf(u - v0[r], v0[r] - l) * 1.000001f : 0.0f;
-        }
-        vref[2 * c] = make_float4(v0[0], v0[1], v0[2], v0[3]);
-        vref[2 * c + 1] = make_float4(dv[0], dv[1], dv[2], dv[3]);
-    }
-}
-
+    vrange_reduce_store(lo, hi, c, vref, red);
+}
+
+__global__ __launch_bounds__(256) void stage_tail_kernel(uint32_t *__restrict__ recs, const uint32_t *__restrict__ grp_start,
+                                                         const uint32_t *__restrict__ grp_cnt, const float *__restrict__ thr,
+                                                         uint32_t opdw, const FactorStats fs, uint32_t tile_images,
+                                                         const float4 *__restrict__ list_uref, float4 *__restrict__ vref) {
+    const uint32_t c = blockIdx.x, n = grp_cnt[c], st0 = grp_start[c];
+    const bool additive = tile_images == 2;
+    const uint32_t opld = rq_img_opld(opdw, additive), img = rq_img_dwords(opdw, additive);
+    const uint32_t taild = additive ? RQ_RECA_TAIL : RQ_REC_TAIL;
+    const float inf = __builtin_inff();
+    float lo[4] = {inf, inf, inf, inf}, hi[4] = {-inf, -inf, -inf, -inf};
+    float4 u0 = make_float4(0.0f, 0.0f, 0.0f, 0.0f);
+    if (additive && n) u0 = list_uref[c];
+    for (uint32_t i = threadIdx.x; i < n; i += 256) {
+        const uint32_t at = st0 + i;
+        uint32_t *base = recs + (uint64_t)(at >> 5) * img + 32 * opld;
+        uint32_t *t = base + (at & 31u) * taild;
+        const uint4 t0 = *reinterpret_cast<const uint4 *>(t), t1 = *reinterpret_cast<const uint4 *>(t + 4);
+        const float lower = __builtin_bit_cast(float, t0.x), delta = __builtin_bit_cast(float, t0.y);
+        const float sumq = __builtin_bit_cast(float, t0.z), ycd = __builtin_bit_cast(float, t0.w);
+        const float ysq = __builtin_bit_cast(float, t1.x);
+        static_assert(RQ_REC_LOWER == 0 && RQ_REC_DELTA == 1 && RQ_REC_SUMQ == 2 && RQ_REC_YCD == 3 && RQ_REC_YCD_SQRT == 4 && RQ_REC_THR == 5,
+                      "the first six tail dwords");
+        const float th = thr[t[RQ_REC_ROW]];
+        t[RQ_REC_THR] = __builtin_bit_cast(uint32_t, th);
+        const StageGate g = stage_gate(lower, delta, sumq, ycd, ysq, th, fs);
+        if (additive) {
+            const float cq = stage_gate_cq(g, sumq, u0);
+            base[32 * RQ_RECA_TAIL + (at & 31u)] = __builtin_bit_cast(uint32_t, cq);
+            if (!(cq < inf)) continue;
+#pragma unroll
+            for (int r = 0; r < 4; ++r) lo[r] = fminf(lo[r], g.v[r]), hi[r] = fmaxf(hi[r], g.v[r]);
+        } else {
+            uint32_t t8[8];
+            stage_gate_bf16(g, sumq, t8);
+            *reinterpret_cast<uint4 *>(t + RQ_REC_V0) = make_uint4(t8[0], t8[1], t8[2], t8[3]);
+            *reinterpret_cast<uint4 *>(t + RQ_REC_V0 + 4) = make_uint4(t8[4], t8[5], t8[6], t8[7]);
+        }
+    }
+    __shared__ float red[4][8];
+    if (additive) vrange_reduce_store(lo, hi, c, vref, red);
+}
+
+struct ClearSpans {
+    uint32_t *p[6];
+    uint32_t n[6];
+};
+__global__ __launch_bounds__(256) void clear_words_kernel(const ClearSpans cs) {
+#pragma unroll
+    for (int j = 0; j < 6; ++j)
+        for (uint32_t i = blockIdx.x * 256 + threadIdx.x; i < cs.n[j]; i += gridDim.x * 256) cs.p[j][i] = 0u;
+}
 
 template <bool FILT>
 __device__ __forceinline__ void scan_generic_body(SCAN_PARAMS, uint32_t W) {
diff --git a/rabitq_amd/csrc/rabitq_hip.hip b/rabitq_amd/csrc/rabitq_hip.hip
--- a/rabitq_amd/csrc/rabitq_hip.hip
+++ b/rabitq_amd/csrc/rabitq_hip.hip
@@ -792,6 +792,11 @@
         g_group_rank = value;
         return RQ_OK;
     }
+    if (std::string(name) == "prep_placement") {
+        if (value < 0 || value > 1) return fail(RQ_ERR_INVALID, "prep_placement must be 0 or 1");
+        g_prep_placement = value;
+        return RQ_OK;
+    }
     if (std::string(name) == "rerank_shadow") {
         if (value < 0 || value > 2) return fail(RQ_ERR_INVALID, "rerank_shadow must be 0 (never), 1 (fp16 rows when they fit) or 2 (8-bit rows when they fit)");
         g_rerank_shadow = value;
```
